# jcfaracco/xpysom-dask

Measured on AMD Instinct MI355X. Metric: samples/sec/epoch, higher is better.
Workload: dtype f16

## Files before the change

### xpysom_dask_amd/_lib.py

```python
import ctypes as C
import importlib.util
import os

HERE = os.path.dirname(os.path.abspath(__file__))
LIB_PATH = os.environ.get("SOM_LIB_PATH") or os.path.join(HERE, "libsomhip.so")

SOM_DIST = {"euclidean": 0, "euclidean_no_opt": 1, "cosine": 2, "manhattan": 3, "manhattan_no_opt": 3,
            "norm_p": 4, "norm_p_no_opt": 5}
SOM_NEIGH = {"gaussian": 0, "mexican_hat": 1, "bubble": 2, "triangle": 3}
SOM_PREC = {"f32": 0, "bf16": 1, "f16": 3, "exact": 5}
SOM_TOPO = {"rectangular": 0, "hexagonal": 1}
SOM_BMU_ACTIVATION, SOM_BMU_QUANTIZATION = 0, 1
SOM_KERNELS = {"bmu": 0, "segsum": 1, "kron": 2, "merge": 3, "prep": 4, "screen": 5}


class SomConfig(C.Structure):
    _fields_ = [("x", C.c_int32), ("y", C.c_int32), ("input_len", C.c_int32),
                ("distance", C.c_int32), ("neighborhood", C.c_int32),
                ("compact_support", C.c_int32), ("precision", C.c_int32), ("device", C.c_int32),
                ("std_coeff", C.c_double), ("stream", C.c_void_p),
                ("topology", C.c_int32), ("norm_p", C.c_int32), ("norm_p_real", C.c_double)]


_F = C.POINTER(C.c_float)
_I = C.POINTER(C.c_int32)
_H = C.c_void_p

SIGNATURES = {
    "som_version": (C.c_char_p, []),
    "som_device_count": (C.c_int, []),
    "som_last_error": (C.c_char_p, [_H]),
    "som_create": (C.c_int, [C.POINTER(SomConfig), C.POINTER(_H)]),
    "som_destroy": (None, [_H]),
    "som_set_weights": (C.c_int, [_H, _F]),
    "som_get_weights": (C.c_int, [_H, _F]),
    "som_set_data": (C.c_int, [_H, _F, C.c_int64]),
    "som_set_data_device": (C.c_int, [_H, C.c_void_p, C.c_int64]),
    "som_sync_producer": (C.c_int, [_H, C.c_uint64, C.c_int32]),
    "som_copy_to_host": (C.c_int, [_H, C.c_void_p, C.c_uint64, C.c_void_p]),
    "som_epoch_accumulate": (C.c_int, [_H, C.c_double, C.c_double, C.c_int]),
    "som_epoch_accumulate_faithful": (C.c_int, [_H, C.c_double, C.c_double, C.c_int]),
    "som_epoch_merge": (C.c_int, [_H]),
    "som_epoch": (C.c_int, [_H, C.c_double, C.c_double, C.c_int]),
    "som_epoch_accumulate_begin": (C.c_int, [_H, C.c_double, C.c_double, C.c_int]),
    "som_epoch_block_count": (C.c_int, [_H, C.POINTER(C.c_int32)]),
    "som_epoch_accumulate_block": (C.c_int, [_H, C.c_int32, C.POINTER(C.c_int64), C.POINTER(C.c_int64)]),
    "som_comm_load": (C.c_int, [C.c_char_p]),
    "som_comm_unique_id": (C.c_int, [C.c_void_p]),
    "som_comm_init": (C.c_int, [_H, C.c_int32, C.c_int32, C.c_void_p]),
    "som_epoch_allreduce": (C.c_int, [_H]),
    "som_comm_destroy": (C.c_int, [_H]),
    "som_pinned_alloc": (C.c_int, [C.c_uint64, C.POINTER(C.c_void_p)]),
    "som_pinned_free": (C.c_int, [C.c_void_p]),
    "som_stream_begin": (C.c_int, [_H]),
    "som_stream_rows": (C.c_int, [_H, _F, C.c_int64]),
    "som_stream_end": (C.c_int, [_H, C.c_double, C.c_double, C.c_int]),
    "som_accum_device_ptr": (C.c_int, [_H, C.POINTER(C.c_void_p), C.POINTER(C.c_int64)]),
    "som_get_stream": (C.c_int, [_H, C.POINTER(C.c_void_p)]),
    "som_epoch_fetch": (C.c_int, [_H, _F, _F, _I]),
    "som_epoch_accumulate_forced": (C.c_int, [_H, _I, C.c_double, C.c_double, C.c_int]),
    "som_bmu": (C.c_int, [_H, _F, C.c_int64, C.c_int32, _I]),
    "som_bmu_device": (C.c_int, [_H, C.c_void_p, C.c_int64, C.c_int32, _I]),
    "som_bmu_top2": (C.c_int, [_H, _F, C.c_int64, _I, _I]),
    "som_bmu_top2_device": (C.c_int, [_H, C.c_void_p, C.c_int64, _I, _I]),
    "som_bmu_f64": (C.c_int, [_H, C.POINTER(C.c_double), C.c_int64, _I]),
    "som_distance_matrix": (C.c_int, [_H, _F, C.c_int64, C.c_int32, _F]),
    "som_quantization_error": (C.c_int, [_H, _F, C.c_int64, C.POINTER(C.c_double)]),
    "som_quantization_error_device": (C.c_int, [_H, C.c_void_p, C.c_int64, C.POINTER(C.c_double)]),
    "som_set_verify": (C.c_int, [_H, C.c_int32]),
    "som_verify_stats": (C.c_int, [_H, C.POINTER(C.c_int64), C.POINTER(C.c_int64)]),
    "som_debug_corrupt_operands": (C.c_int, [_H, C.c_int32]),
    "som_debug_operand_crc": (C.c_int, [_H, C.c_int32, C.POINTER(C.c_uint64)]),
    "som_debug_exact_centroids": (C.c_int, [_H, C.c_int32, _F, _F, _F, _I]),
    "som_debug_mfma16": (C.c_int, [_H, C.c_void_p, C.c_void_p, _F, _F, C.c_int32]),
    "som_debug_stamps": (C.c_int, [_H, C.c_int64, C.c_void_p]),
    "som_debug_device_bytes": (C.c_int, [C.POINTER(C.c_int64)]),
    "som_debug_qe_stats": (C.c_int, [_H, C.POINTER(C.c_int64), C.POINTER(C.c_int64)]),
    "som_debug_exact_chain_stats": (C.c_int, [_H, C.POINTER(C.c_int64)]),
    "som_debug_exact_select_stats": (C.c_int, [_H, C.POINTER(C.c_int64), C.POINTER(C.c_int64), C.POINTER(C.c_int64)]),
    "som_policy_eval": (C.c_int, [C.c_int32, C.POINTER(C.c_double), C.POINTER(C.c_double), C.POINTER(C.c_int32)]),
    "som_policy_replay": (C.c_int, [C.c_int32, C.POINTER(C.c_double), C.POINTER(C.c_double)]),
    "som_patch_order": (C.c_int, [C.c_int32, C.c_int32, _I]),
    "som_exact_stats": (C.c_int, [_H, C.POINTER(C.c_int64), C.POINTER(C.c_int64), C.POINTER(C.c_int64)]),
    "som_exact_top2_stats": (C.c_int, [_H, C.POINTER(C.c_int64), C.POINTER(C.c_int64)]),
    "som_exact_skip_stats": (C.c_int, [_H, C.POINTER(C.c_int64), C.POINTER(C.c_int64)]),
    "som_exact_resident_stats": (C.c_int, [_H, C.POINTER(C.c_int64), C.POINTER(C.c_int64)]),
    "som_exact_scout_stats": (C.c_int, [_H, C.POINTER(C.c_int64), C.POINTER(C.c_int64)]),
    "som_exact_refine_stats": (C.c_int, [_H, C.POINTER(C.c_int64), C.POINTER(C.c_int64)]),
    "som_exact_last_counts": (C.c_int, [_H, _I, C.c_int64]),
    "som_sync": (C.c_int, [_H]),
    "som_profile_enable": (C.c_int, [_H, C.c_int32]),
    "som_profile_get": (C.c_int, [_H, C.c_int32, C.POINTER(C.c_double), C.POINTER(C.c_int64)]),
    "som_profile_reset": (C.c_int, [_H]),
}

_lib = None


def torch_lib_file(name):
    try:
        spec = importlib.util.find_spec("torch")
    except (ImportError, ValueError):
        spec = None
    if spec is None or not spec.submodule_search_locations:
        return None
    cand = os.path.join(list(spec.submodule_search_locations)[0], "lib", name)
    return cand if os.path.exists(cand) else None


def _preload_torch_hip_runtime():
    try:
        spec = importlib.util.find_spec("torch")
    except (ImportError, ValueError):
        spec = None
    if spec is None or not spec.submodule_search_locations:
        return
    cand = os.path.join(list(spec.submodule_search_locations)[0], "lib", "libamdhip64.so")
    if os.path.exists(cand):
        try:
            C.CDLL(cand, mode=C.RTLD_GLOBAL)
        except OSError:
            pass


def load():
    global _lib
    if _lib is not None:
        return _lib
    if not os.path.exists(LIB_PATH):
        raise ImportError(
            f"{LIB_PATH} is missing: build it with `python -m xpysom_dask_amd.build` "
            "(needs hipcc; there is no CPU fallback)")
    if not os.environ.get("SOM_LIB_PATH"):
        from . import build as _build
        have, want = _build.built_hash(LIB_PATH), _build.source_hash()
        if have != want:
            raise ImportError(
                f"{LIB_PATH} is stale: built from sources {have}, the tree is {want}; "
                "rebuild with `python -m xpysom_dask_amd.build`")
    _preload_torch_hip_runtime()
    lib = C.CDLL(LIB_PATH)
    for name, (res, args) in SIGNATURES.items():
        fn = getattr(lib, name)
        fn.restype = res
        fn.argtypes = args
    _lib = lib
    return lib
```

### xpysom_dask_amd/csrc/exact_host.hpp

```cpp

struct PassCtr {
    int* base; int n_groups; bool whole_lines;
    int* gcount() const { return base; }
    int* gstart() const { return base + n_groups; }
    PassCounters* tail() const { return (PassCounters*)(gstart() + n_groups); }
    RowNeed* row_need() const { return (RowNeed*)base; }
    size_t bytes() const {
        const size_t b = 2 * (size_t)n_groups * sizeof(int) + sizeof(PassCounters);
        return whole_lines ? (size_t)round_up((long)b, 64) : b;
    }
};
constexpr size_t EX_CTR_TAIL_INTS = (sizeof(PassCounters) + 64) / sizeof(int);
inline PassCtr pass_ctr(const som_handle* h) { return PassCtr{h->ex.ctr, (int)cdiv(h->K, EX_GROUP), h->ex.chain}; }

constexpr double EX_KAPPA = 6.0;
ExactBound exact_bound(const som_handle* h) {
    const double u = std::ldexp(1.0, -24);
    const double Dl = h->wide ? 32.0 * h->ft_kchunks : 8.0 * h->fr_kg;
    const double n_mfma = h->wide ? h->n_kchunks : h->ks32;
    const double gamma = Dl * u / (1.0 - Dl * u);
    const double slop = 1.01;
    ExactBound eb{};
    eb.cB = (float)(slop * 2.0 * (EX_KAPPA * n_mfma + 1.0) * std::ldexp(1.0, -23));
    eb.cM = (float)(slop * 2.0);
// ... 244 lines not shown
    ex.tile_counts.reset(); ex.tlist.reset(); ex.tcnt.reset(); ex.scout_g.reset(); ex.items.reset(); ex.tile_ticket.reset();
    ex.sk_stride = 0;
    const long tiles = stride / SK_TILE;
    if (int rc = ex.sk_keys.alloc(h, (size_t)stride)) return rc;
    if (int rc = ex.sk_keys2.alloc(h, (size_t)stride)) return rc;
    if (int rc = ex.sk_vals.alloc(h, (size_t)stride)) return rc;
    if (int rc = ex.scout_g.alloc(h, (size_t)stride)) return rc;
    if (h->wide)
        if (int rc = ex.tq.alloc(h, (size_t)stride)) return rc;
    if (int rc = ex.need.alloc(h, (size_t)tiles * ex.cen[0].n_cstages)) return rc;
    if (int rc = ex.need2.alloc(h, (size_t)tiles * ex.cen[1].n_cstages)) return rc;
    if (int rc = ex.glist.alloc(h, (size_t)tiles * n_groups)) return rc;
    if (int rc = ex.gcnt.alloc(h, (size_t)tiles)) return rc;
    if (int rc = ex.tile_counts.alloc(h, (size_t)tiles)) return rc;
    if (int rc = ex.tlist.alloc(h, (size_t)tiles * n_groups * K16_T)) return rc;
    if (int rc = ex.tcnt.alloc(h, (size_t)tiles)) return rc;
    if (int rc = ex.tile_ticket.alloc(h, (size_t)tiles)) return rc;
    ex.item_slots = (int)resident_slots(h, 8);
    if (int rc = ex.items.alloc(h, (size_t)(5 * tiles + 4 * ex.item_slots + 16))) return rc;
    if (int rc = ex.sk_tmp.alloc(h, radix_scratch_ints(stride))) return rc;
    ex.sk_stride = stride;
    return 0;
}

template <class E>
int exact_skip_centroids(som_handle* h, const float* xmax2, unsigned q_blocks, unsigned long long* best64, long n_rows, bool* q_done) {
    auto& ex = h->ex;
    const float* Wsrc = h->ex_patch ? h->Wp : h->W;
    const int n_groups = (int)cdiv(h->K, EX_GROUP);
    auto& c0 = ex.cen[0];
    auto& c1 = ex.cen[1];
    const CentroidLevel l1{c0.Cc, c0.rg, c0.csq, c0.cmax2, c0.n_slots}, l2{c1.Cc, c1.rg, c1.csq, c1.cmax2, c1.n_slots};
    if (!ex.cen_fresh)
        exact_centroids_kernel<<<dim3((unsigned)(cdiv(n_groups, 4) * 4)), dim3(512), 0, h->stream>>>(Wsrc, h->K, h->D, n_groups, l1, l2, h->wmax2);
    const int nst2 = ex.lp.level2 ? c1.n_cstages : 0;
    char* plain = ex.lp.scout ? c0.Cst_plain : nullptr;
    const dim3 tgrid((unsigned)cdiv((long)(c0.n_cstages + nst2) * K16_T, 4)), block(256);
    if (ex.prep_w_pending) {
        ex.prep_w_pending = false;
        const float* Wex = h->ex_patch ? h->Wp : h->W;
        float* cm1 = ex.prep_w_cm ? (float*)c0.cmax2 : nullptr;
        float* cm2 = ex.prep_w_cm ? (float*)c1.cmax2 : nullptr;
        const unsigned w_blocks = (unsigned)cdiv((long)h->n_stages * K16_T, 4);
        switch (h->ks32) {
#define SOM_PIMG_CASE(k) case k: exact_prep_images_kernel<k, E><<<dim3(w_blocks + tgrid.x + q_blocks), block, 0, h->stream>>>(w_blocks, tgrid.x, Wex, h->K, h->D, h->Wst, h->n_stages, \
            h->wmax2 + 1, h->Wst_lo, cm1, cm2, l1, c0.Cst, c0.n_cstages, l2, c1.Cst, nst2, xmax2, h->wmax2, plain, h->wn, h->stage_units, best64, n_rows); break;
        SOM_PIMG_CASE(1) SOM_PIMG_CASE(2) SOM_PIMG_CASE(3) SOM_PIMG_CASE(4)
#undef SOM_PIMG_CASE
        default: return fail(h, "exact: block skipping supports input_len <= 128");
        }
        HIPCHK(h, hipGetLastError());
        *q_done = q_blocks > 0;
        return 0;
    }
    switch (h->ks32) {
#define SOM_CIMG_CASE(k) case k: exact_centroid_image_kernel<k, E><<<tgrid, block, 0, h->stream>>>(l1, c0.Cst, c0.n_cstages, l2, c1.Cst, nst2, h->D, xmax2, h->wmax2, plain); break;
    SOM_CIMG_CASE(1) SOM_CIMG_CASE(2) SOM_CIMG_CASE(3) SOM_CIMG_CASE(4)
#undef SOM_CIMG_CASE
    default: return fail(h, "exact: block skipping supports input_len <= 128");
    }
    HIPCHK(h, hipGetLastError());
    return 0;
}

int exact_skip_sortkeys(som_handle* h, som_handle::ExactScratch::SortedRows& sr, long s0, long n, const int* prev, const int* scout_g) {
    auto& ex = h->ex;
    const int n_groups = (int)cdiv(h->K, EX_GROUP);
    if (scout_g != nullptr)
        exact_groupkey_kernel<<<dim3((unsigned)cdiv(n, 256)), dim3(256), 0, h->stream>>>(scout_g, n, n_groups, ex.sk_keys, ex.sk_vals);
    else
        exact_sortkey_kernel<<<dim3((unsigned)cdiv(n, 256)), dim3(256), 0, h->stream>>>(prev, h->ex_inv, n, h->K, ex.sk_keys, ex.sk_vals);
    int bits = 1;
    while ((1L << bits) < n_groups) ++bits;
    return radix_sort_rows(h, ex.sk_keys, n, bits, ex.sk_keys2, sr.order + s0, ex.sk_tmp);
}
template <class E>
int exact_skip_gather(som_handle* h, som_handle::ExactScratch::SortedRows& sr, long s0, const int* order, const float* X, const __bf16* Xb, long n,
                      const float* xsq, const float* xerr, const float* xmax2) {
    const long np = round_up(n, SK_TILE);
    exact_gather_sorted_kernel<E><<<dim3((unsigned)cdiv(np, 16)), dim3(256), 0, h->stream>>>(
        order, n, np, h->dp, h->D, Xb, X, xsq, xerr, xmax2, sr.Xb_s + s0 * h->dp, sr.Xl_s != nullptr ? sr.Xl_s + s0 * h->dp : nullptr, sr.Xf_s + s0 * h->D,
        sr.xsq_s + s0, sr.xerr_s + s0);
    HIPCHK(h, hipGetLastError());
    return 0;
}

template <int KS32, class E>
int exact_scout_nearest_ks(som_handle* h, const __bf16* Xb, long n, unsigned long long* best64, int* g_out) {
    auto& ex = h->ex;
    const auto& c0 = ex.cen[0];
    const void* kern = (const void*)bmu_bf16_k16_kernel<KS32, E, false, false>;
    const size_t lds = 2 * (size_t)k16_stage_bytes(KS32);
    int per_cu = 1;
    if (int rc = kernel_per_cu(h, kern, 64 * K16_NW, lds, &per_cu)) return rc;
    const long blocks = cdiv(n, K16_WG_SAMPLES);
    const long slots = resident_slots(h, per_cu);
    const int parts = std::max(1, std::min(choose_parts(h, blocks, slots, c0.n_cstages), c0.n_cstages));
    bmu_bf16_k16_kernel<KS32, E, false, false><<<dim3((unsigned)blocks, (unsigned)parts), dim3(64 * K16_NW), lds, h->stream>>>(
        Xb, n, c0.Cst_plain, c0.n_cstages, c0.n_slots, best64);
    bmu_finalize_kernel<<<dim3((unsigned)cdiv(n, 256)), dim3(256), 0, h->stream>>>(best64, n, c0.n_slots, g_out);
    HIPCHK(h, hipMemsetAsync(best64, 0xFF, (size_t)n * sizeof(unsigned long long), h->stream));
    HIPCHK(h, hipGetLastError());
    return 0;
}
template <class E>
int exact_scout_nearest(som_handle* h, const __bf16* Xb, long n, unsigned long long* best64, int* g_out) {
    SOM_KS32_DISPATCH(exact_scout_nearest_ks, h, Xb, n, best64, g_out)
    return fail(h, "exact: the scout supports input_len <= 128");
}

template <int KS32, class E>
int exact_scout_pick_ks(som_handle* h, som_handle::ExactScratch::SortedRows& sr, long s0, long n, const int* keys, unsigned long long* best64) {
    auto& ex = h->ex;
    const int n_groups = (int)cdiv(h->K, EX_GROUP);
    const long tiles = round_up(n, SK_TILE) / SK_TILE;
    const size_t lds_l = (size_t)cdiv(n_groups, 64) * sizeof(unsigned long long);
    exact_scout_lists_kernel<<<dim3((unsigned)tiles), dim3(64), lds_l, h->stream>>>(keys, nullptr, n, n_groups, ex.tlist, ex.tcnt);
    const void* kern = (const void*)bmu_bf16_k16_kernel<KS32, E, false, true>;
    const size_t lds = 2 * (size_t)k16_stage_bytes(KS32);
    int per_cu = 1;
    if (int rc = kernel_per_cu(h, kern, 64 * K16_NW, lds, &per_cu)) return rc;
    bmu_bf16_k16_kernel<KS32, E, false, true><<<dim3((unsigned)tiles, 1), dim3(64 * K16_NW), lds, h->stream>>>(
        sr.Xb_s + s0 * h->dp, n, h->Wst, h->n_stages, h->K, best64, nullptr, 0, nullptr, nullptr, nullptr, nullptr, nullptr, nullptr, ExactBound(),
        nullptr, ex.tlist, ex.tcnt);
    exact_scout_pos_kernel<<<dim3((unsigned)cdiv(n, 256)), dim3(256), 0, h->stream>>>(best64, n, h->K, sr.lastpos_s + s0);
    HIPCHK(h, hipGetLastError());
    return 0;
}
template <class E>
int exact_scout_pick(som_handle* h, som_handle::ExactScratch::SortedRows& sr, long s0, long n, const int* keys, unsigned long long* best64) {
    SOM_KS32_DISPATCH(exact_scout_pick_ks, h, sr, s0, n, keys, best64)
    return fail(h, "exact: the scout supports input_len <= 128");
}

void exact_plan_lists(som_handle* h, long tiles, int n_cstages, const unsigned long long* need2) {
    auto& ex = h->ex;
    const int n_groups = (int)cdiv(h->K, EX_GROUP);
    PassCounters* const ctr = pass_ctr(h).tail();
    const int slots = ex.item_queue ? (ex.screen_slots > 0 ? ex.screen_slots : ex.item_slots) : 0;
    int2* const queue = ex.item_queue ? ex.items + 8 : nullptr;
    int* const n_items = (int*)ex.items.p;
    if (ex.chain) {
        exact_lists_totals_kernel<<<dim3((unsigned)cdiv(tiles, LISTS_WG_TILES)), dim3(64 * LISTS_WG_TILES), 0, h->stream>>>(
            ex.need, n_cstages, need2, n_groups, ex.glist, ex.gcnt, ex.tile_counts, ex.tlist, ex.tcnt, tiles, &ctr->lists_done,
            &ctr->blocks_run, &ctr->groups_run, slots, queue, n_items, n_items + 1, ex.item_len_pct, ex.tile_ticket);
        return;
    }
    exact_lists_kernel<<<dim3((unsigned)tiles), dim3(64), 0, h->stream>>>(ex.need, n_cstages, need2, n_groups, ex.glist, ex.gcnt,
                                                                         ex.tile_counts, ex.tlist, ex.tcnt, ex.tile_ticket);
    exact_list_totals_kernel<<<dim3(1), dim3(1024), 0, h->stream>>>(ex.tile_counts, tiles, &ctr->blocks_run, &ctr->groups_run, slots, queue,
                                                                  n_items, n_items + 1, ex.item_len_pct);
}

template <class E>
int exact_skip_plan(som_handle* h, som_handle::ExactScratch::SortedRows& sr, long s0, long n, const float* xmax2, const ExactBound& eb,
                    const int* lastpos2, bool time_l2 = false) {
    auto& ex = h->ex;
    PassCounters* const ctr = pass_ctr(h).tail();
    const long np = round_up(n, SK_TILE);
    const long tiles = np / SK_TILE;
    const dim3 block(64 * K16_NW);
    const auto& c0 = ex.cen[0];
    const auto& c1 = ex.cen[1];
    const long want = (1024 + tiles - 1) / tiles;
    const dim3 pgrid((unsigned)tiles, (unsigned)std::max<long>(1, std::min<long>({want, 4L, (long)c0.n_cstages})));
    const size_t lds1 = 2 * (size_t)h->stage_bytes + (size_t)c0.n_cstages * 8;
    const size_t lds2 = 2 * (size_t)h->stage_bytes + (size_t)c0.n_cstages * 64 * sizeof(int) + (size_t)c1.n_cstages * 8;
    const bool l2 = ex.lp.level2;
    const int force = ex.skip_mode == 3 ? 1 : 0;
    const __bf16* Xs = sr.Xb_s + s0 * h->dp;
    unsigned long long* const need2_clear = l2 && ex.chain ? ex.need2.p : nullptr;
    if (l2 && !ex.chain) HIPCHK(h, hipMemsetAsync(ex.need2, 0, (size_t)tiles * c1.n_cstages * sizeof(unsigned long long), h->stream));
#define SOM_PLAN_CASE(k) case k: { \
        { int pc; if (int rc = kernel_per_cu(h, (const void*)exact_plan_kernel<k, E, false>, 64 * K16_NW, lds1, &pc)) return rc; } \
        exact_plan_kernel<k, E, false><<<pgrid, block, lds1, h->stream>>>(Xs, n, c0.Cst, c0.n_cstages, c0.rg, c0.n_slots, \
            sr.xsq_s + s0, sr.xerr_s + s0, sr.sU_s + s0, xmax2, c0.cmax2, h->wmax2, h->wmax2 + 1, eb, ex.need, sr.lastpos_s + s0, \
            h->Wst, sr.seed_s + s0, nullptr, 0, force, lastpos2, lastpos2 != nullptr ? &ctr->scout_wins : nullptr, need2_clear); \
        if (l2) { \
            if (time_l2) (void)hipEventRecord(ex.cost.ev[3], h->stream); \
            { int pc; if (int rc = kernel_per_cu(h, (const void*)exact_plan_kernel<k, E, true>, 64 * K16_NW, lds2, &pc)) return rc; } \
            exact_plan_kernel<k, E, true><<<dim3((unsigned)tiles, pgrid.y), block, lds2, h->stream>>>(Xs, n, c1.Cst, c1.n_cstages, c1.rg, c1.n_slots, \
                sr.xsq_s + s0, sr.xerr_s + s0, sr.sU_s + s0, xmax2, c1.cmax2, h->wmax2, h->wmax2 + 1, eb, ex.need2, nullptr, \
                nullptr, nullptr, ex.need, c0.n_cstages, force); \
            if (time_l2) (void)hipEventRecord(ex.cost.ev[4], h->stream); \
        } } break;
    switch (h->ks32) {
    SOM_PLAN_CASE(1) SOM_PLAN_CASE(2) SOM_PLAN_CASE(3) SOM_PLAN_CASE(4)
    default: return fail(h, "exact: block skipping supports input_len <= 128");
    }
#undef SOM_PLAN_CASE
    exact_plan_lists(h, tiles, c0.n_cstages, l2 ? ex.need2.p : nullptr);
    HIPCHK(h, hipGetLastError());
    return 0;
}

template <class E>
int exact_wide_centroids(som_handle* h, const float* xmax2) {
    auto& ex = h->ex;
    auto& c0 = ex.cen[0];
    const float* Wsrc = h->ex_patch ? h->Wp : h->W;
    const int n_groups = (int)cdiv(h->K, EX_GROUP);
    wide_centroids_kernel<<<dim3((unsigned)n_groups), dim3(256), 0, h->stream>>>(Wsrc, h->K, h->D, n_groups, c0.Cc, c0.rg, c0.csq, c0.cmax2, h->wmax2);
    const long total = (long)c0.n_img_stages * WD_T * h->n_kchunks * 64;
    prep_w_bf16_wide_kernel<E><<<dim3((unsigned)cdiv(total, 256)), dim3(256), 0, h->stream>>>(c0.Cc, n_groups, h->D, h->n_kchunks, c0.Cst, c0.n_img_stages,
                                                                                             nullptr, h->wmax2);
    exact_werr_kernel<E><<<dim3((unsigned)cdiv(n_groups, 4 * EX_WERR_UNITS)), dim3(256), 0, h->stream>>>(c0.Cc, n_groups, h->D, h->wmax2, c0.cmax2 + 1, nullptr);
    char* plain = ex.lp.scout ? c0.Cst_plain : nullptr;
    if (plain) HIPCHK(h, hipMemcpyAsync(plain, c0.Cst, (size_t)c0.n_img_stages * h->stage_bytes, hipMemcpyDeviceToDevice, h->stream));
    wide_centroid_tail_kernel<<<dim3((unsigned)cdiv((long)c0.n_img_stages * WD_STAGE_UNITS, 256)), dim3(256), 0, h->stream>>>(
        c0.rg, c0.csq, n_groups, c0.Cst, c0.n_img_stages, h->stage_bytes, xmax2, h->wmax2, plain);
    HIPCHK(h, hipGetLastError());
    return 0;
}

template <class E>
int exact_wide_gather(som_handle* h, som_handle::ExactScratch::SortedRows& sr, long s0, const float* X, long n, const float* xsq, const float* xerr,
                      const int* prev, const float* xmax2) {
    const long np = round_up(n, SK_TILE);
    wide_gather_sorted_kernel<<<dim3((unsigned)cdiv(np, 4)), dim3(256), 0, h->stream>>>(sr.order + s0, n, np, h->D, X, xsq, xerr, prev,
                                                                                      sr.Xf_s + s0 * h->D, sr.xsq_s + s0, sr.xerr_s + s0, sr.lastpos_s + s0);
    const long n_blocks = np / h->tl_bm;
    const long total = n_blocks * h->n_kchunks * (h->tl_bm / 16) * TL_KS * 64;
    prep_tiles_bf16_kernel<E><<<dim3((unsigned)cdiv(total, 256)), dim3(256), 0, h->stream>>>(
        sr.Xf_s + s0 * h->D, n, h->D, h->n_kchunks, n_blocks, h->tl_bm, h->tl_xtile, 1.0f, nullptr, (char*)(sr.Xb_s + s0 * h->dp), xmax2);
    HIPCHK(h, hipGetLastError());
    return 0;
}

template <int KS32, class E>
int exact_wide_scout_nearest_ks(som_handle* h, const __bf16* Ximg, long n, unsigned long long* best64, int* g_out) {
    auto& ex = h->ex;
    const auto& c0 = ex.cen[0];
    const size_t lds = (size_t)WD_SLOTS * wd_stage_bytes(KS32);
    int per_cu = 1;
    if (int rc = kernel_per_cu(h, (const void*)bmu_bf16_wide_kernel<KS32, E>, 64 * WD_NW, lds, &per_cu)) return rc;
    const long blocks = cdiv(n, WD_WG_SAMPLES);
    const long slots = resident_slots(h, per_cu);
    const int parts = (int)std::max<long>(1, std::min<long>({cdiv(2 * slots, blocks), 8L, (long)c0.n_img_stages}));
    bmu_bf16_wide_kernel<KS32, E><<<dim3((unsigned)blocks, (unsigned)parts), dim3(64 * WD_NW), lds, h->stream>>>(
        (const char*)Ximg, n, c0.Cst_plain, c0.n_img_stages, best64);
    bmu_finalize_kernel<<<dim3((unsigned)cdiv(n, 256)), dim3(256), 0, h->stream>>>(best64, n, c0.n_slots, g_out);
    HIPCHK(h, hipMemsetAsync(best64, 0xFF, (size_t)n * sizeof(unsigned long long), h->stream));
    HIPCHK(h, hipGetLastError());
    return 0;
}
template <int KS32, class E>
int exact_wide_scout_pick_ks(som_handle* h, som_handle::ExactScratch::SortedRows& sr, long s0, long n, const int* keys, unsigned long long* best64) {
    auto& ex = h->ex;
    const int n_groups = (int)cdiv(h->K, EX_GROUP);
    const long tiles = round_up(n, SK_TILE) / SK_TILE;
    const size_t lds_l = (size_t)cdiv(n_groups, 64) * sizeof(unsigned long long);
    exact_scout_lists_kernel<<<dim3((unsigned)tiles), dim3(64), lds_l, h->stream>>>(keys, nullptr, n, n_groups, ex.glist, ex.gcnt, 1);
    const size_t lds = (size_t)WD_SLOTS * wd_stage_bytes(KS32);
    int per_cu = 1;
    if (int rc = kernel_per_cu(h, (const void*)bmu_bf16_wide_kernel<KS32, E, false, true>, 64 * WD_NW, lds, &per_cu)) return rc;
    bmu_bf16_wide_kernel<KS32, E, false, true><<<dim3((unsigned)tiles, 1), dim3(64 * WD_NW), lds, h->stream>>>(
        (const char*)(sr.Xb_s + s0 * h->dp), n, h->Wst, h->n_stages, best64, nullptr, 0, nullptr, nullptr, nullptr, nullptr, nullptr, nullptr, ExactBound(),
        ex.glist, ex.gcnt, n_groups);
    exact_scout_pos_kernel<<<dim3((unsigned)cdiv(n, 256)), dim3(256), 0, h->stream>>>(best64, n, h->K, sr.lastpos_s + s0, h->ex_perm);
    HIPCHK(h, hipGetLastError());
    return 0;
}
template <class E>
int exact_wide_scout_nearest(som_handle* h, const __bf16* Ximg, long n, unsigned long long* best64, int* g_out) {
    SOM_WIDE_DISPATCH(exact_wide_scout_nearest_ks, h, Ximg, n, best64, g_out)
    return fail(h, "exact: no wide scout instance for this input_len");
}
template <class E>
int exact_wide_scout_pick(som_handle* h, som_handle::ExactScratch::SortedRows& sr, long s0, long n, const int* keys, unsigned long long* best64) {
    SOM_WIDE_DISPATCH(exact_wide_scout_pick_ks, h, sr, s0, n, keys, best64)
    return fail(h, "exact: no wide scout instance for this input_len");
}

template <int KS32, class E>
int exact_wide_plan_ks(som_handle* h, som_handle::ExactScratch::SortedRows& sr, long s0, long n, const float* xmax2, const ExactBound& eb) {
    auto& ex = h->ex;
    const auto& c0 = ex.cen[0];
    const long np = round_up(n, SK_TILE);
    const long tiles = np / SK_TILE;
    exact_seed_kernel<<<dim3((unsigned)cdiv(n * 16, 256)), dim3(256), 0, h->stream>>>(
        sr.Xf_s + s0 * h->D, n, h->D, h->W, h->wsq, h->K, sr.lastpos_s + s0, sr.xsq_s + s0, sr.xerr_s + s0, h->wmax2, xmax2, h->wmax2 + 1, eb, ex.seed, ex.tq);
    wide_plan_rows_kernel<<<dim3((unsigned)cdiv(n, 256)), dim3(256), 0, h->stream>>>(n, sr.xsq_s + s0, sr.xerr_s + s0, ex.tq, xmax2, c0.cmax2, h->wmax2,
                                                                                  h->wmax2 + 1, eb, ex.skip_mode == 3 ? 1 : 0, sr.seed_s + s0, sr.sU_s + s0);
    HIPCHK(h, hipMemsetAsync(ex.need, 0, (size_t)tiles * c0.n_cstages * sizeof(unsigned long long), h->stream));
    auto kern = bmu_bf16_wide_kernel<KS32, E, false, false, true>;
    const size_t lds = (size_t)WD_SLOTS * wd_stage_bytes(KS32) + (size_t)c0.n_cstages * sizeof(unsigned long long);
    int per_cu = 1;
    if (int rc = kernel_per_cu(h, (const void*)kern, 64 * WD_NW, lds, &per_cu)) return rc;
    const long slots = resident_slots(h, per_cu);
    int parts = (int)std::max<long>(1, std::min<long>({cdiv(2 * slots, tiles), 8L, (long)c0.n_img_stages}));
    bmu_bf16_wide_kernel<KS32, E, false, false, true><<<dim3((unsigned)tiles, (unsigned)parts), dim3(64 * WD_NW), lds, h->stream>>>(
        (const char*)(sr.Xb_s + s0 * h->dp), n, c0.Cst, c0.n_img_stages, nullptr, nullptr, 0, nullptr, nullptr, nullptr, nullptr, nullptr, nullptr, ExactBound(),
        nullptr, nullptr, 0, sr.seed_s + s0, sr.sU_s + s0, ex.need, c0.n_cstages);
    exact_plan_lists(h, tiles, c0.n_cstages, nullptr);
    HIPCHK(h, hipGetLastError());
    return 0;
}
template <class E>
int exact_wide_plan(som_handle* h, som_handle::ExactScratch::SortedRows& sr, long s0, long n, const float* xmax2, const ExactBound& eb) {
    SOM_WIDE_DISPATCH(exact_wide_plan_ks, h, sr, s0, n, xmax2, eb)
    return fail(h, "exact: no wide plan instance for this input_len");
}

template <int KG>
int exact_rescore_kg(som_handle* h, const float* X, unsigned long long* best64, int deint) {
    auto& ex = h->ex;
    auto kern = exact_rescore_mfma_kernel<KG>;
    const size_t lds = (size_t)fr_stage_bytes(KG);
    int per_cu = 1;
    if (int rc = kernel_per_cu(h, (const void*)kern, 256, lds, &per_cu)) return rc;
    const long grid = std::min<long>(ex.max_tiles, h->ex.grid_mult * resident_slots(h, per_cu));
    kern<<<dim3((unsigned)grid), dim3(256), lds, h->stream>>>(X, h->D, h->Wfst, h->K, ex.tile_tab, &pass_ctr(h).tail()->n_tiles, ex.plist,
                                                             best64, h->ex_perm, nullptr, h->ex_sub44 ? 1 : 0, deint, nullptr);
    return 0;
}

inline unsigned exact_tiles_blocks(const som_handle* h) { return h->ex.chain ? 16u : 1u; }

template <int KS32, class E>
int exact_refine_ks(som_handle* h, som_handle::ExactScratch::SortedRows& sr, long r0, long n, const float* xmax2, const ExactBound& eb) {
    auto& ex = h->ex;
    const PassCtr pc = pass_ctr(h);
    const int n_groups = pc.n_groups;
// ... 385 lines not shown
```

### xpysom_dask_amd/csrc/exact_skip.hpp

```cpp
#pragma once
#include "bmu_bf16_k16.hpp"
#include "bmu_f32_res.hpp"

namespace somhip {

constexpr int SK_TILE = K16_WG_SAMPLES;
static_assert(K16_STAGE_UNITS == 64 && K16_T == 4, "block skipping: a stage of the resident screen is one 64-unit group of four 16-unit tiles");

struct CentroidLevel { float* C; float* rg; float* csq; float* cmax2; int n_slots; };
struct CentroidShared {
    float qsum[4][128];
    float part[2][64][2];
    float csq_s[2][5];
};
__device__ __forceinline__ void group_centroids(const float (&w)[16], int g, int K, int D, const CentroidLevel& l1,
                                                const CentroidLevel& l2, CentroidShared& sh) {
    const int tid = threadIdx.x, lane = tid & 63;
    const int d = tid & 127, q = tid >> 7, fh = (tid >> 6) & 1;
    const int cnt = (int)max(0L, min(64L, (long)K - (long)g * 64));
    const int cb = max(0, min(16, cnt - 16 * q));
    float sum = 0.0f;
#pragma unroll
    for (int k = 0; k < 16; ++k) sum += w[k];
    sh.qsum[q][d] = sum;
// ... 156 lines not shown

template <class EL>
__global__ __launch_bounds__(256) void exact_gather_sorted_kernel(const int* __restrict__ order, long n, long np, int dp, int D,
                                                                  const __bf16* __restrict__ Xb, const float* __restrict__ X,
                                                                  const float* __restrict__ xsq, const float* __restrict__ xerr,
                                                                  const float* __restrict__ xmax2,
                                                                  __bf16* __restrict__ Xb_s, __bf16* __restrict__ Xl_s,
                                                                  float* __restrict__ Xf_s,
                                                                  float* __restrict__ xsq_s, float* __restrict__ xerr_s) {
    using E = typename EL::T;
    using bf16x8 = typename V8<E>::t;
    const int lane = threadIdx.x & 15;
    const long p = (long)blockIdx.x * 16 + (threadIdx.x >> 4);
    if (p >= np) return;
    const long r = p < n ? (long)order[p] : -1;
    const float sx = ex_scale(*xmax2);
    const bool vec = (D & 7) == 0;
    for (int c = lane; c < dp / 8; c += 16) {
        bf16x8 v, vl;
#pragma unroll
        for (int j = 0; j < 8; ++j) { v[j] = (E)0.0f; vl[j] = (E)0.0f; }
        if (r >= 0) {
            v = *(const bf16x8*)((const char*)Xb + (r * dp + c * 8) * 2);
            float f[8];
            if (vec && c * 8 < D) {
                const f32x4 a = *(const f32x4*)(X + r * D + c * 8), b = *(const f32x4*)(X + r * D + c * 8 + 4);
                const f32x4 ev = {a[0], a[2], b[0], b[2]}, od = {a[1], a[3], b[1], b[3]};
                *(f32x4*)(Xf_s + p * D + c * 4) = ev;
                *(f32x4*)(Xf_s + p * D + D / 2 + c * 4) = od;
#pragma unroll
                for (int j = 0; j < 4; ++j) { f[j] = a[j]; f[4 + j] = b[j]; }
            } else {
#pragma unroll
                for (int j = 0; j < 8; ++j) {
                    f[j] = c * 8 + j < D ? X[r * D + c * 8 + j] : 0.0f;
                    if (c * 8 + j < D) Xf_s[p * D + c * 8 + j] = f[j];
                }
            }
#pragma unroll
            for (int j = 0; j < 8; ++j) {
                const float d = (f[j] * sx - (float)v[j]) * 2048.0f;
                vl[j] = cvt<E>(d == d && __builtin_fabsf(d) < 3.0e38f ? d : 0.0f);
            }
        }
        *(bf16x8*)((char*)Xb_s + (p * dp + c * 8) * 2) = v;
        if (Xl_s != nullptr) *(bf16x8*)((char*)Xl_s + (p * dp + c * 8) * 2) = vl;
    }
    if (lane == 0) {
        const float nanv = __builtin_nanf("");
        xsq_s[p] = r >= 0 ? xsq[r] : nanv;
        xerr_s[p] = r >= 0 ? xerr[r] : nanv;
    }
}

__device__ __forceinline__ float up_to_half(float v) {
    if (!(v == v)) return v;
    if (v > 65504.0f) return __builtin_inff();
    if (v < 0x1p-14f) return 0x1p-14f;
    const _Float16 hv = (_Float16)v;
    float f = (float)hv;
    if (f < v) f = (float)__builtin_bit_cast(_Float16, (unsigned short)(__builtin_bit_cast(unsigned short, hv) + 1));
    return f;
}

__device__ __forceinline__ uint32_t row16_or(uint32_t v) {
    v |= (uint32_t)__builtin_amdgcn_update_dpp(0, (int)v, 0x121, 0xF, 0xF, false);
    v |= (uint32_t)__builtin_amdgcn_update_dpp(0, (int)v, 0x122, 0xF, 0xF, false);
    v |= (uint32_t)__builtin_amdgcn_update_dpp(0, (int)v, 0x124, 0xF, 0xF, false);
    v |= (uint32_t)__builtin_amdgcn_update_dpp(0, (int)v, 0x128, 0xF, 0xF, false);
    return v;
}

template <int KS32, class EL>
__device__ __forceinline__ void exact_centroid_image_body(const unsigned bid, const CentroidLevel& l1, char* __restrict__ Cst1, int n_cstages1,
                                                          const CentroidLevel& l2, char* __restrict__ Cst2, int n_cstages2, int D,
                                                          const float* __restrict__ xmax2, const float* __restrict__ wmax2,
                                                          char* __restrict__ Cst1_plain) {
    using E = typename EL::T;
    using bf16x8 = typename V8<E>::t;
    constexpr int STAGE = k16_stage_bytes(KS32);
    const int lane = threadIdx.x & 63;
    long tile = (long)bid * 4 + (threadIdx.x >> 6);
    const long t1 = (long)n_cstages1 * K16_T;
    const bool second = tile >= t1;
    if (second) tile -= t1;
    if (tile >= (long)(second ? n_cstages2 : n_cstages1) * K16_T) return;
    const CentroidLevel& lv = second ? l2 : l1;
    char* Cst = second ? Cst2 : Cst1;
    const long stage = tile / K16_T;
    const int t16 = (int)(tile - stage * K16_T);
    const long slot = stage * K16_STAGE_UNITS + t16 * 16 + (lane & 15);
    const float sw = ex_scale(*wmax2), sx = ex_scale(*xmax2);
    float er = 0.0f;
#pragma unroll
    for (int ks = 0; ks < KS32; ++ks) {
        const int k0 = ks * 32 + (lane >> 4) * 8;
        bf16x8 v;
#pragma unroll
        for (int j = 0; j < 8; ++j) {
            const float f = (slot < lv.n_slots && k0 + j < D) ? lv.C[slot * D + k0 + j] * sw : 0.0f;
            const E hb = cvt<E>(-f);
            v[j] = hb;
            const float e = half_operand_error(-f, (float)hb);
            er = __builtin_fmaf(e, e, er);
        }
        *(bf16x8*)(Cst + stage * STAGE + ((long)(t16 * KS32 + ks) * 64 + lane) * 16) = v;
        if (!second && Cst1_plain != nullptr) *(bf16x8*)(Cst1_plain + stage * STAGE + ((long)(t16 * KS32 + ks) * 64 + lane) * 16) = v;
    }
    er += __shfl_xor(er, 16, 64);
    er += __shfl_xor(er, 32, 64);
    float m = (er == er) ? er : 0.0f;
#pragma unroll
    for (int o = 8; o > 0; o >>= 1) m = fmaxf(m, __shfl_xor(m, o, 64));
    if (lane == 0) atomic_max_pos_f32(lv.cmax2 + 1, m);
    if (lane < 16) {
        float* tail = (float*)(Cst + (stage + 1) * (long)STAGE - 1024);
        const int within = t16 * 16 + lane;
        const float rad = slot < lv.n_slots ? lv.rg[slot] : -1.0f;
        float* ptail = (!second && Cst1_plain != nullptr) ? (float*)(Cst1_plain + (stage + 1) * (long)STAGE - 1024) : nullptr;
        if (rad < 0.0f) { tail[within] = __builtin_inff(); tail[64 + within] = 0.0f; if (ptail) ptail[within] = __builtin_inff(); }
        else {
            const float big = __builtin_sqrtf(*wmax2) * __builtin_sqrtf(*xmax2) * (1.0f + 1.0f / 1024.0f);
            const float S = sx * sw, hS = 0.5f * S * (1.0f + 1.0f / 1024.0f);
            const float s0 = __builtin_fmaf(0.5f * S, lv.csq[slot], S * big);
            tail[within] = s0 - hS * rad * rad * (1.0f + 0x1p-20f);
            tail[64 + within] = -up_to_half(sw * rad);
            if (ptail) ptail[within] = (s0 == s0 && s0 < 3.0e38f) ? s0 : __builtin_inff();
        }
    }
}
template <int KS32, class EL>
__global__ __launch_bounds__(256) void exact_centroid_image_kernel(CentroidLevel l1, char* __restrict__ Cst1, int n_cstages1,
                                                                   CentroidLevel l2, char* __restrict__ Cst2, int n_cstages2, int D,
                                                                   const float* __restrict__ xmax2, const float* __restrict__ wmax2,
                                                                   char* __restrict__ Cst1_plain = nullptr) {
    exact_centroid_image_body<KS32, EL>(blockIdx.x, l1, Cst1, n_cstages1, l2, Cst2, n_cstages2, D, xmax2, wmax2, Cst1_plain);
}

template <int KS32, class EL>
__global__ __launch_bounds__(256) void exact_prep_images_kernel(unsigned w_blocks, unsigned c_blocks, const float* __restrict__ W, int K, int D,
                                                                char* __restrict__ Wst, int n_stages, float* __restrict__ werr2,
                                                                char* __restrict__ Wst_lo, float* __restrict__ cm1, float* __restrict__ cm2,
                                                                CentroidLevel l1, char* __restrict__ Cst1, int n_cstages1,
                                                                CentroidLevel l2, char* __restrict__ Cst2, int n_cstages2,
                                                                const float* __restrict__ xmax2, const float* __restrict__ wmax2,
                                                                char* __restrict__ Cst1_plain, const float* __restrict__ wn,
                                                                int stage_units, unsigned long long* __restrict__ best64, long n_rows) {
    if (blockIdx.x < w_blocks) prep_w_exact_k16_body<KS32, EL>(blockIdx.x, W, K, D, Wst, n_stages, wmax2, werr2, Wst_lo, cm1, cm2, false);
    else if (blockIdx.x < w_blocks + c_blocks)
        exact_centroid_image_body<KS32, EL>(blockIdx.x - w_blocks, l1, Cst1, n_cstages1, l2, Cst2, n_cstages2, D, xmax2, wmax2, Cst1_plain);
    else prep_wsqh_body(blockIdx.x - w_blocks - c_blocks, wn, K, wmax2, xmax2, Wst, n_stages, k16_stage_bytes(KS32), stage_units, best64, n_rows, 1);
}

template <int KS32, class EL, bool LEVEL2>
__global__ __launch_bounds__(64 * K16_NW, LEVEL2 ? 3 : 2) void exact_plan_kernel(const __bf16* __restrict__ Xb, long N,
                                                                    const char* __restrict__ Cst, int n_cstages,
                                                                    const float* __restrict__ rg, int n_slots,
                                                                    const float* __restrict__ xsq, const float* __restrict__ xerr,
                                                                    float* __restrict__ sU_s,
                                                                    const float* __restrict__ xmax2, const float* __restrict__ cmax2,
                                                                    const float* __restrict__ wmax2, const float* __restrict__ werr2,
                                                                    ExactBound eb, unsigned long long* __restrict__ need,
                                                                    const int* __restrict__ lastpos, const char* __restrict__ Wst,
                                                                    float* __restrict__ seed_s,
                                                                    const unsigned long long* __restrict__ need1, int n_cstages1,
                                                                    int force_all, const int* __restrict__ lastpos2 = nullptr,
                                                                    int* __restrict__ scout_wins = nullptr,
                                                                    unsigned long long* __restrict__ need2_clear = nullptr) {
    using E = typename EL::T;
    using bf16x8 = typename V8<E>::t;
    constexpr int DP = 32 * KS32;
    constexpr int STAGE = k16_stage_bytes(KS32);
    constexpr int PIECES = K16_T * KS32 + 1;
    extern __shared__ __attribute__((aligned(16))) char smem[];
    __shared__ int act_n;

    const int tid = threadIdx.x, lane = tid & 63;
    const int wave = __builtin_amdgcn_readfirstlane(tid >> 6);
    const int quad = lane >> 4, col = lane & 15;
    const long wave_s0 = (long)blockIdx.x * K16_WG_SAMPLES + wave * (16 * K16_SB);

    bf16x8 xf[K16_SB][KS32];
    bf16x8 xe[K16_SB];
    float A[K16_SB], sU[K16_SB], P[K16_SB];
    const ExactScales sc = ex_scales(xmax2, cmax2, cmax2 + 1);
    const ExactScales sw = ex_scales(xmax2, wmax2, werr2);
    const float S = sc.sx * sc.sw;
#pragma unroll
    for (int sb = 0; sb < K16_SB; ++sb) {
        const long row = wave_s0 + sb * 16 + col;
#pragma unroll
        for (int ks = 0; ks < KS32; ++ks) xf[sb][ks] = *(const bf16x8*)(Xb + row * DP + ks * 32 + quad * 8);
        A[sb] = -__builtin_inff(); sU[sb] = 0.0f;
        if (row < N) {
            const float q = xsq[row], xe = xerr[row];
            float su;
            if (!LEVEL2) {
                auto value_of = [&](int pos) -> float {
                    const char* stg = Wst + (long)(pos >> 6) * STAGE;
                    const int t16 = (pos >> 4) & 3, c = pos & 15;
                    float d = 0.0f;
#pragma unroll
                    for (int ks = 0; ks < KS32; ++ks) {
                        const bf16x8 a = *(const bf16x8*)(stg + ((t16 * KS32 + ks) * 64 + quad * 16 + c) * 16);
#pragma unroll
                        for (int jj = 0; jj < 8; ++jj) d = __builtin_fmaf((float)a[jj], (float)xf[sb][ks][jj], d);
                    }
                    d += __shfl_xor(d, 16, 64);
                    d += __shfl_xor(d, 32, 64);
                    return *(const float*)(stg + K16_T * KS32 * 1024 + (t16 * 16 + c) * 4) + d;
                };
                float vu = value_of(lastpos[row]);
                if (lastpos2 != nullptr) {
                    const float v2 = value_of(lastpos2[row]);
                    const float Sq = sw.sx * sw.sw;
                    const float ua = q + 2.0f * (vu / Sq - sw.big), ub = q + 2.0f * (v2 / Sq - sw.big);
                    const bool win = ua < 0.9f * ub;
                    const unsigned long long wm = __ballot(win && quad == 0);
                    if (scout_wins != nullptr && lane == __builtin_ctzll(__ballot(true)) && wm != 0ull) atomicAdd(scout_wins, (int)__popcll(wm));
                    vu = (v2 < vu || !(vu == vu)) ? v2 : vu;
                }
                const float Sw = sw.sx * sw.sw;
                const float e = ex_row_bound(eb, sw, q, xe);
                const float f32s = ex_f32_share(eb, sw, q);
                const float e_valu = 48.0f * 0x1p-24f * Sw * sw.bmag;
                const float sd = vu + (e - f32s) * (1.0f + 1.0f / 1024.0f) + e_valu + Sw * sw.bmag * 0x1p-21f;
                if (quad == 0) seed_s[row] = (sd > 0.0f && sd < 3.0e38f) ? sd : __builtin_inff();
                const float e_one = 0.5f * (e - f32s) * (1.0f + 1.0f / 1024.0f) + e_valu;
                const float tau_up = 2.0f * (((vu + e_one) - Sw * sw.big) / Sw) + 0x1p-20f * (sw.big + __builtin_fabsf(vu) / Sw);
                const float xn = __builtin_sqrtf(q) * (1.0f + 1.0f / 1024.0f);
                const float share = 2.0f * (eb.cA * xn * sw.wm + eb.cW * sw.wm * sw.wm);
                const float U0 = q * (1.0f + 1.0f / 1024.0f) + tau_up + share * (1.0f + 1.0f / 1024.0f) + 0x1p-18f * (q + __builtin_fabsf(tau_up));
                const float U = U0 < 0.0f ? 0.0f : U0;
                su = __builtin_sqrtf(U) * (1.0f + 1.0f / 1024.0f);
                if (force_all || !(su == su) || !(su < 3.0e38f) || !(e == e)) su = __builtin_inff();
                if (quad == 0) sU_s[row] = su;
            } else {
                su = sU_s[row];
            }
            const float ec = 0.5f * ex_row_bound(eb, sc, q, xe) * (1.0f + 1.0f / 1024.0f);
            sU[sb] = su;
            A[sb] = S * sc.big + ec - 0.5f * S * q * (1.0f - 1.0f / 1024.0f) + 0x1p-12f * S * (sc.big + q) + 0x1p-16f * S * sc.wm * sc.wm;
            if (!(A[sb] == A[sb]) || !(A[sb] < 3.0e38f) || !(su < 3.0e38f)) {
                A[sb] = __builtin_inff(); sU[sb] = 0.0f;
            }
        }
        const float bx = up_to_half(sc.sx * sU[sb] * (1.0f + 1.0f / 1024.0f));
        P[sb] = A[sb] + 0.5f * S * (1.0f + 1.0f / 1024.0f) * sU[sb] * sU[sb] * (1.0f + 0x1p-20f) + (float)(24 * (KS32 + 1)) * 0x1p-23f * S * sc.bmag;
        if (!(bx < 3.0e38f) || !(P[sb] == P[sb])) P[sb] = __builtin_inff();
        if (A[sb] == -__builtin_inff()) P[sb] = -__builtin_inff();
#pragma unroll
        for (int jj = 0; jj < 8; ++jj) xe[sb][jj] = (E)0.0f;
        if (quad == 0 && bx < 3.0e38f) xe[sb][0] = (E)bx;
    }

    int* act = (int*)(smem + 2 * STAGE);
    unsigned long long* nl = (unsigned long long*)(smem + 2 * STAGE + (LEVEL2 ? (size_t)n_cstages1 * 64 * sizeof(int) : 0));
    for (int i = tid; i < n_cstages; i += 64 * K16_NW) nl[i] = 0ull;
    if constexpr (LEVEL2) {
        static_assert(K16_NW == 4, "a wave per tile fills the slot's tail");
        if (wave == 0) {
            int cnt = 0;
            for (int s1 = 0; s1 < n_cstages1; ++s1) {
                const unsigned long long w = need1[(long)blockIdx.x * n_cstages1 + s1];
                const int g = s1 * 64 + lane;
                const bool on = ((w >> lane) & 1ull) && 4 * (g >> 2) * 4 < n_slots;
                const unsigned long long mk = __ballot(on);
                if (on) act[cnt + __popcll(mk & ((1ull << lane) - 1ull))] = g;
                cnt += __popcll(mk);
            }
            if (lane == 0) act_n = cnt;
        }
        __syncthreads();
        const int n_act = act_n;
        const int c_all = (n_act + 15) / 16;
        const int b0 = 16 * (int)((long)c_all * blockIdx.y / gridDim.y);
        const int e0 = min(n_act, 16 * (int)((long)c_all * (blockIdx.y + 1) / gridDim.y));
        constexpr int TQ = K16_T * KS32 * 1024;
        auto frag_of = [&](int g, int sub, int ks, int q) -> const char* {
            return Cst + (long)(g >> 4) * STAGE + (((((g >> 2) & 3) * KS32 + ks) * 64 + q * 16 + 4 * (g & 3) + sub) * 16);
        };
        auto dma_chunk = [&](int c0, char* dst) {
            for (int p = wave; p < K16_T * KS32; p += K16_NW) {
                const int j = p / KS32, ks = p - j * KS32;
                if (c0 + 4 * j < e0) {
                    const int gi = c0 + 4 * j + (col >> 2);
                    const int g = gi < e0 ? act[gi] : act[c0 + 4 * j];
                    lds_dma_16(frag_of(g, col & 3, ks, quad), dst + p * 1024);
                }
            }
        };
        auto load_tail = [&](int c0) -> float {
            const int i = lane & 15, gi = c0 + 4 * wave + (i >> 2);
            if (lane >= 32 || gi >= e0) return lane < 16 ? __builtin_inff() : 0.0f;
            const int g = act[gi];
            return *(const float*)(Cst + (long)(g >> 4) * STAGE + TQ + (((lane >> 4) * 64) + ((g >> 2) & 3) * 16 + 4 * (g & 3) + (i & 3)) * 4);
        };
        auto store_tail = [&](char* dst, float v) {
            if (lane < 32) *(float*)(dst + TQ + (((lane >> 4) * 64) + wave * 16 + (lane & 15)) * 4) = v;
        };
        if (b0 < e0) { dma_chunk(b0, smem); store_tail(smem, load_tail(b0)); }
        int k = 0;
        for (int c0 = b0; c0 < e0; c0 += 16, ++k) {
            asm volatile("s_waitcnt vmcnt(0) lgkmcnt(0)" ::: "memory");
            __builtin_amdgcn_s_barrier();
            asm volatile("" ::: "memory");
            char* sn = smem + ((k + 1) & 1) * STAGE;
            float tail_n = 0.0f;
            if (c0 + 16 < e0) { dma_chunk(c0 + 16, sn); tail_n = load_tail(c0 + 16); }
            const char* st = smem + (k & 1) * STAGE;
            const float* wq = (const float*)(st + TQ);
            auto load_tile = [&](int j, bf16x8 (&a)[KS32], f32x4& wv, float& rneg) {
#pragma unroll
                for (int ks = 0; ks < KS32; ++ks) a[ks] = *(const bf16x8*)(st + ((j * KS32 + ks) * 64 + lane) * 16);
                wv = *(const f32x4*)(wq + j * 16 + 4 * quad);
                rneg = wq[64 + j * 16 + col];
            };
            uint32_t lane_bits = 0u;
            auto run_tile = [&](int j, const bf16x8 (&a)[KS32], const f32x4& wv, float rneg) {
                bf16x8 ae;
#pragma unroll
                for (int jj = 0; jj < 8; ++jj) ae[jj] = (E)0.0f;
                if (quad == 0) ae[0] = (E)rneg;
                f32x4 acc[K16_SB];
#pragma unroll
                for (int sb = 0; sb < K16_SB; ++sb) acc[sb] = wv;
#pragma unroll
                for (int ks = 0; ks < KS32; ++ks)
#pragma unroll
                    for (int sb = 0; sb < K16_SB; ++sb) acc[sb] = mfma16(a[ks], xf[sb][ks], acc[sb]);
#pragma unroll
                for (int sb = 0; sb < K16_SB; ++sb) acc[sb] = mfma16(ae, xe[sb], acc[sb]);
#pragma unroll
                for (int r = 0; r < 4; ++r) {
                    bool nd = false;
#pragma unroll
                    for (int sb = 0; sb < K16_SB; ++sb) nd = nd || !(acc[sb][r] > P[sb]);
                    lane_bits |= nd ? (1u << (4 * j + r)) : 0u;
                }
            };
            bf16x8 aA[KS32], aB[KS32];
            f32x4 wvA, wvB;
            float rnA, rnB;
            const bool h1 = c0 + 4 < e0, h2 = c0 + 8 < e0, h3 = c0 + 12 < e0;
            load_tile(0, aA, wvA, rnA);
            if (h1) load_tile(1, aB, wvB, rnB);
            run_tile(0, aA, wvA, rnA);
            if (h1) {
                if (h2) load_tile(2, aA, wvA, rnA);
                run_tile(1, aB, wvB, rnB);
                if (h2) {
                    if (h3) load_tile(3, aB, wvB, rnB);
                    run_tile(2, aA, wvA, rnA);
                    if (h3) run_tile(3, aB, wvB, rnB);
                }
            }
            const uint32_t any_row = row16_or(lane_bits);
            if (col == 0 && any_row != 0u) {
#pragma unroll
                for (int j = 0; j < 4; ++j) {
                    const uint32_t nib = (any_row >> (4 * j)) & 15u;
                    const int gi = c0 + 4 * j + quad;
                    if (nib != 0u && gi < e0) {
                        const int g = act[gi];
                        atomicOr(nl + (g >> 4), (unsigned long long)nib << (4 * (g & 15)));
                    }
                }
            }
            if (c0 + 16 < e0) store_tail(sn, tail_n);
        }
        __syncthreads();
        for (int i = tid; i < n_cstages; i += 64 * K16_NW)
            if (nl[i] != 0ull) atomicOr(need + (long)blockIdx.x * n_cstages + i, nl[i]);
        return;
    }
    const int n_walk = n_cstages;
    const int s_begin = (int)((long)n_walk * blockIdx.y / gridDim.y);
    const int s_end = (int)((long)n_walk * (blockIdx.y + 1) / gridDim.y);
    auto item_of = [&](int i) -> int { return (i << 4) | 15; };
    auto dma_stage = [&](int s, uint32_t tm, char* dst) {
        const char* src = Cst + (long)s * STAGE;
        for (int p = wave; p < PIECES; p += K16_NW)
            if (p == PIECES - 1 || ((tm >> (p / KS32)) & 1u)) lds_dma_16(src + (long)p * 1024 + lane * 16, dst + p * 1024);
    };
    int st_cur = 0, st_next = 0;
    uint32_t tm_cur = 0, tm_next = 0;
    if (s_begin < s_end) {
        const int it = item_of(s_begin);
        st_cur = it >> 4; tm_cur = (uint32_t)it & 15u;
        dma_stage(st_cur, tm_cur, smem);
    }
    for (int i = s_begin; i < s_end; ++i) {
        asm volatile("s_waitcnt vmcnt(0) lgkmcnt(0)" ::: "memory");
        __builtin_amdgcn_s_barrier();
        asm volatile("" ::: "memory");
        if (i + 1 < s_end) {
            const int it = item_of(i + 1);
            st_next = it >> 4; tm_next = (uint32_t)it & 15u;
            dma_stage(st_next, tm_next, smem + ((i + 1 - s_begin) & 1) * STAGE);
        }
        const char* st = smem + ((i - s_begin) & 1) * STAGE;
        const float* wq = (const float*)(st + K16_T * KS32 * 1024);
        uint32_t lane_bits = 0u;
        auto load_tile = [&](int t, bf16x8 (&a)[KS32], f32x4& wv, float& rneg) {
#pragma unroll
            for (int ks = 0; ks < KS32; ++ks) a[ks] = *(const bf16x8*)(st + ((t * KS32 + ks) * 64 + lane) * 16);
            wv = *(const f32x4*)(wq + t * 16 + 4 * quad);
            rneg = wq[64 + t * 16 + col];
        };
        auto run_tile = [&](int t16, const bf16x8 (&a)[KS32], const f32x4& wv, float rneg) {
            bf16x8 ae;
#pragma unroll
            for (int jj = 0; jj < 8; ++jj) ae[jj] = (E)0.0f;
            if (quad == 0) ae[0] = (E)rneg;
            f32x4 acc[K16_SB];
#pragma unroll
            for (int sb = 0; sb < K16_SB; ++sb) acc[sb] = wv;
#pragma unroll
            for (int ks = 0; ks < KS32; ++ks)
#pragma unroll
                for (int sb = 0; sb < K16_SB; ++sb) acc[sb] = mfma16(a[ks], xf[sb][ks], acc[sb]);
#pragma unroll
            for (int sb = 0; sb < K16_SB; ++sb) acc[sb] = mfma16(ae, xe[sb], acc[sb]);
#pragma unroll
            for (int r = 0; r < 4; ++r) {
                bool nd = false;
#pragma unroll
                for (int sb = 0; sb < K16_SB; ++sb) nd = nd || !(acc[sb][r] > P[sb]);
                lane_bits |= nd ? (1u << (4 * t16 + r)) : 0u;
            }
        };
        const uint32_t m0 = 15u, m1 = m0 & (m0 - 1u), m2 = m1 & (m1 - 1u), m3 = m2 & (m2 - 1u);
        const int t0 = __builtin_ctz(m0), t1 = m1 ? __builtin_ctz(m1) : -1, t2 = m2 ? __builtin_ctz(m2) : -1, t3 = m3 ? __builtin_ctz(m3) : -1;
        bf16x8 aA[KS32], aB[KS32];
        f32x4 wvA, wvB;
        float rnA, rnB;
        load_tile(t0, aA, wvA, rnA);
        if (t1 >= 0) load_tile(t1, aB, wvB, rnB);
        run_tile(t0, aA, wvA, rnA);
        if (t1 >= 0) {
            if (t2 >= 0) load_tile(t2, aA, wvA, rnA);
            run_tile(t1, aB, wvB, rnB);
            if (t2 >= 0) {
                if (t3 >= 0) load_tile(t3, aB, wvB, rnB);
                run_tile(t2, aA, wvA, rnA);
                if (t3 >= 0) run_tile(t3, aB, wvB, rnB);
            }
        }
        const uint32_t any_row = row16_or(lane_bits);
        if (col == 0 && any_row != 0u) {
            const uint32_t lo = ((any_row & 15u) | (((any_row >> 4) & 15u) << 16)) << (4 * quad);
            const uint32_t hi = (((any_row >> 8) & 15u) | (((any_row >> 12) & 15u) << 16)) << (4 * quad);
            atomicOr(nl + (i - s_begin), ((unsigned long long)hi << 32) | lo);
        }
        st_cur = st_next; tm_cur = tm_next;
    }
    __syncthreads();
    for (int i = s_begin + tid; i < s_end; i += 64 * K16_NW) need[(long)blockIdx.x * n_cstages + i] = nl[i - s_begin];
    if (need2_clear != nullptr)
        for (int i = 4 * s_begin + tid; i < 4 * s_end; i += 64 * K16_NW) need2_clear[(long)blockIdx.x * 4 * n_cstages + i] = 0ull;
}

template <bool PUBLISH>
__device__ __forceinline__ void exact_lists_tile(const long tile, const int lane, const unsigned long long* __restrict__ need1, int n_cstages,
                                                 const unsigned long long* __restrict__ need2, int n_groups,
                                                 int* __restrict__ glist, int* __restrict__ gcnt,
                                                 int2* tile_counts, int* __restrict__ tlist,
                                                 int* __restrict__ tcnt, int* __restrict__ tile_ticket) {
    const unsigned long long below = (1ull << lane) - 1ull;
    int base = 0, blk = 0, kept = 0;
    for (int s0 = 0; s0 < n_cstages; s0 += 64) {
        const unsigned long long mine = s0 + lane < n_cstages ? need1[tile * n_cstages + s0 + lane] : 0ull;
        const uint32_t lo = (uint32_t)mine, hi = (uint32_t)(mine >> 32);
        unsigned long long todo = __ballot(mine != 0ull);
        for (; todo != 0ull; todo &= todo - 1ull) {
            const int sl = (int)__builtin_ctzll(todo), s = s0 + sl;
            const unsigned long long w = ((unsigned long long)(uint32_t)__builtin_amdgcn_readlane((int)hi, sl) << 32) |
                                         (uint32_t)__builtin_amdgcn_readlane((int)lo, sl);
            uint32_t nib = 15u;
            if (need2 != nullptr) nib = (uint32_t)(need2[tile * 4 * n_cstages + 4 * s + (lane >> 4)] >> (4 * (lane & 15))) & 15u;
            const int g = s * 64 + lane;
            const bool l1 = ((w >> lane) & 1ull) && g < n_groups;
            const bool on = l1 && nib != 0u;
            const unsigned long long mk = __ballot(on);
            if (on) glist[tile * n_groups + base + __popcll(mk & ((1ull << lane) - 1ull))] = (g << 4) | (int)nib;
            base += __popcll(mk);
            kept += __popcll(__ballot(l1));
            int before = 0, total = 0;
#pragma unroll
            for (int b = 0; b < 4; ++b) {
                const unsigned long long mb = __ballot(on && ((nib >> b) & 1u));
                before += __popcll(mb & below);
                total += __popcll(mb);
            }
            if (on) {
                int o = blk + before;
#pragma unroll
                for (int b = 0; b < 4; ++b)
                    if ((nib >> b) & 1u) tlist[tile * 4 * n_groups + o++] = (g << 2) | b;
            }
            blk += total;
        }
    }
    if (lane == 0) {
        gcnt[tile] = base; tcnt[tile] = blk;
        tile_ticket[tile] = 0;
        if (PUBLISH)
            __hip_atomic_store((unsigned long long*)(tile_counts + tile), ((unsigned long long)(uint32_t)kept << 32) | (uint32_t)blk,
                               __ATOMIC_RELAXED, __HIP_MEMORY_SCOPE_AGENT);
        else tile_counts[tile] = make_int2(blk, kept);
    }
}
__global__ __launch_bounds__(64) void exact_lists_kernel(const unsigned long long* __restrict__ need1, int n_cstages,
                                                         const unsigned long long* __restrict__ need2, int n_groups,
                                                         int* __restrict__ glist, int* __restrict__ gcnt,
                                                         int2* __restrict__ tile_counts, int* __restrict__ tlist,
                                                         int* __restrict__ tcnt, int* __restrict__ tile_ticket) {
    exact_lists_tile<false>(blockIdx.x, threadIdx.x, need1, n_cstages, need2, n_groups, glist, gcnt, tile_counts, tlist, tcnt, tile_ticket);
}

__device__ __forceinline__ void exact_list_totals_body(const int2* tile_counts, long tiles, int* __restrict__ blocks_run,
                                                       int* __restrict__ groups_run, int slots, int2* __restrict__ items,
                                                       int* __restrict__ n_items, int* __restrict__ item_ctr, int len_pct,
                                                       int* sb, int* sk, int& tot_b) {
    const int tid = threadIdx.x, lane = tid & 63, wave = tid >> 6;
    int b = 0, k = 0;
    for (long t = tid; t < tiles; t += 1024) { const int2 c = tile_counts[t]; b += c.x; k += c.y; }
#pragma unroll
    for (int o = 32; o > 0; o >>= 1) { b += __shfl_xor(b, o, 64); k += __shfl_xor(k, o, 64); }
    if (lane == 0) { sb[wave] = b; sk[wave] = k; }
    __syncthreads();
    if (tid == 0) {
        b = 0; k = 0;
        for (int w = 0; w < 16; ++w) { b += sb[w]; k += sk[w]; }
        *blocks_run = b; *groups_run = k;
        tot_b = b;
    }
    if (items == nullptr) return;
    __syncthreads();
    const long total = tot_b;
    const long by_mean = (len_pct * total) / (100 * (tiles > 0 ? tiles : 1)) + 1, by_slots = total / (2 * (long)(slots > 0 ? slots : 1));
    const int L = (int)max(32L, min(by_mean, by_slots));
    auto parts_of = [&](int cnt) -> int { return cnt <= L ? 1 : (cnt + L - 1) / L; };
    const long per = (tiles + 1023) / 1024, t_b = min((long)tid * per, tiles), t_e = min(t_b + per, tiles);
    int mine = 0;
    for (long t = t_b; t < t_e; ++t) mine += parts_of(tile_counts[t].x);
    int incl = mine;
#pragma unroll
    for (int o = 1; o < 64; o <<= 1) { const int v = __shfl_up(incl, o, 64); if (lane >= o) incl += v; }
    __syncthreads();
    if (lane == 63) sb[wave] = incl;
    __syncthreads();
    int before = 0, all = 0;
#pragma unroll
    for (int w = 0; w < 16; ++w) { if (w < wave) before += sb[w]; all += sb[w]; }
    int o = before + incl - mine;
    for (long t = t_b; t < t_e; ++t) {
        const int np = parts_of(tile_counts[t].x);
        for (int q = 0; q < np; ++q) items[o++] = make_int2((int)t, q | (np << 16));
    }
    if (tid == 0) { *n_items = all; *item_ctr = 0; }
}
__global__ __launch_bounds__(1024) void exact_list_totals_kernel(const int2* __restrict__ tile_counts, long tiles, int* __restrict__ blocks_run,
                                                                 int* __restrict__ groups_run, int slots = 0, int2* __restrict__ items = nullptr,
                                                                 int* __restrict__ n_items = nullptr, int* __restrict__ item_ctr = nullptr,
                                                                 int len_pct = 125) {
    __shared__ int sb[16], sk[16];
    __shared__ int tot_b;
    exact_list_totals_body(tile_counts, tiles, blocks_run, groups_run, slots, items, n_items, item_ctr, len_pct, sb, sk, tot_b);
}

constexpr int LISTS_WG_TILES = 16;
__global__ __launch_bounds__(64 * LISTS_WG_TILES) void exact_lists_totals_kernel(const unsigned long long* __restrict__ need1, int n_cstages,
                                                                                const unsigned long long* __restrict__ need2, int n_groups,
                                                                                int* __restrict__ glist, int* __restrict__ gcnt,
                                                                                int2* tile_counts, int* __restrict__ tlist,
                                                                                int* __restrict__ tcnt, long tiles, int* __restrict__ done,
                                                                                int* __restrict__ blocks_run, int* __restrict__ groups_run,
                                                                                int slots, int2* __restrict__ items, int* __restrict__ n_items,
                                                                                int* __restrict__ item_ctr, int len_pct,
                                                                                int* __restrict__ tile_ticket) {
    static_assert(LISTS_WG_TILES == 16, "the totals' scan is written for sixteen waves");
    __shared__ int sb[16], sk[16];
    __shared__ int tot_b;
    __shared__ int last;
    const int tid = threadIdx.x;
    const long tile = (long)blockIdx.x * LISTS_WG_TILES + (tid >> 6);
    if (tile < tiles) exact_lists_tile<true>(tile, tid & 63, need1, n_cstages, need2, n_groups, glist, gcnt, tile_counts, tlist, tcnt, tile_ticket);
    asm volatile("s_waitcnt vmcnt(0)" ::: "memory");
    __syncthreads();
    if (tid == 0) {
        const int ticket = __hip_atomic_fetch_add(done, 1, __ATOMIC_RELAXED, __HIP_MEMORY_SCOPE_AGENT);
        last = ticket == (int)gridDim.x - 1 ? 1 : 0;
        if (last) {
            __builtin_amdgcn_fence(__ATOMIC_ACQUIRE, "agent");
            asm volatile("s_waitcnt vmcnt(0)" ::: "memory");
            __hip_atomic_store(done, 0, __ATOMIC_RELAXED, __HIP_MEMORY_SCOPE_AGENT);
        }
    }
    __syncthreads();
    if (!last) return;
    exact_list_totals_body(tile_counts, tiles, blocks_run, groups_run, slots, items, n_items, item_ctr, len_pct, sb, sk, tot_b);
}

__global__ __launch_bounds__(256) void exact_groupkey_kernel(const int* __restrict__ g, long n, int n_groups, int* __restrict__ keys,
                                                             int* __restrict__ vals) {
    const long i = (long)blockIdx.x * 256 + threadIdx.x;
    if (i >= n) return;
    const int v = g[i];
    keys[i] = v < 0 ? 0 : v >= n_groups ? n_groups - 1 : v;
    vals[i] = (int)i;
}

__global__ __launch_bounds__(64) void exact_scout_lists_kernel(const int* __restrict__ gkey, const int* __restrict__ lastpos, long n,
                                                               int n_groups, int* __restrict__ tlist, int* __restrict__ tcnt,
                                                               int group_items = 0) {
    extern __shared__ unsigned long long sbm[];
    const long tile = blockIdx.x;
    const int lane = threadIdx.x;
    const int nw = (n_groups + 63) / 64;
    for (int w = lane; w < nw; w += 64) sbm[w] = 0ull;
    __syncthreads();
    for (int i = 0; i < SK_TILE / 64; ++i) {
        const long p = tile * SK_TILE + i * 64 + lane;
        if (p < n) {
            int g = gkey[p];
            g = g < 0 ? 0 : g >= n_groups ? n_groups - 1 : g;
            atomicOr(sbm + (g >> 6), 1ull << (g & 63));
            if (lastpos != nullptr) {
                int g2 = lastpos[p] >> 6;
                g2 = g2 < 0 ? 0 : g2 >= n_groups ? n_groups - 1 : g2;
                atomicOr(sbm + (g2 >> 6), 1ull << (g2 & 63));
            }
        }
    }
    __syncthreads();
    int base = 0;
    int* out = tlist + tile * (group_items ? 1 : 4) * (long)n_groups;
    for (int w0 = 0; w0 < nw; w0 += 64) {
        unsigned long long word = w0 + lane < nw ? sbm[w0 + lane] : 0ull;
        const int c = __popcll(word);
        int incl = c;
#pragma unroll
        for (int o = 1; o < 64; o <<= 1) { const int t = __shfl_up(incl, o, 64); if (lane >= o) incl += t; }
        int at = base + incl - c;
        for (; word != 0ull; word &= word - 1ull) {
            const int g = (w0 + lane) * 64 + (int)__builtin_ctzll(word);
            if (group_items) out[at] = (g << 4) | 15;
            else {
#pragma unroll
                for (int b = 0; b < 4; ++b) out[4 * at + b] = (g << 2) | b;
            }
            ++at;
        }
        base += __shfl(incl, 63, 64);
    }
    if (lane == 0) tcnt[tile] = group_items ? base : 4 * base;
}

__global__ __launch_bounds__(256) void exact_scout_rowneed_kernel(const float* __restrict__ X, long N, int D, int n_samples,
                                                                  const float* __restrict__ Cc, const float* __restrict__ rg,
                                                                  int n_groups, int* __restrict__ counts) {
    extern __shared__ float xs[];
    __shared__ float wmin[4];
    __shared__ int wcnt[4];
    const int tid = threadIdx.x, lane = tid & 63, wave = tid >> 6;
    const long step = N / n_samples;
    const float* x = X + ((long)blockIdx.x * step + step / 2) * D;
    for (int k = tid; k < D; k += 256) xs[k] = x[k];
    __syncthreads();
    auto dist = [&](int g) -> float {
        const float* c = Cc + (long)g * D;
        float q = 0.0f;
        if ((D & 3) == 0) {
            for (int k = 0; k < D; k += 4) {
                const f32x4 v = *(const f32x4*)(c + k);
#pragma unroll
                for (int j = 0; j < 4; ++j) { const float t = xs[k + j] - v[j]; q = __builtin_fmaf(t, t, q); }
            }
        } else {
            for (int k = 0; k < D; ++k) { const float t = xs[k] - c[k]; q = __builtin_fmaf(t, t, q); }
        }
        return __builtin_sqrtf(q);
    };
    float m = __builtin_inff();
    for (int g = tid; g < n_groups; g += 256) {
        const float r = rg[g];
        if (r >= 0.0f) m = __builtin_fminf(m, dist(g) + r);
    }
#pragma unroll
    for (int o = 32; o > 0; o >>= 1) m = __builtin_fminf(m, __shfl_xor(m, o, 64));
    if (lane == 0) wmin[wave] = m;
    __syncthreads();
    m = __builtin_fminf(__builtin_fminf(wmin[0], wmin[1]), __builtin_fminf(wmin[2], wmin[3]));
    int need = 0;
    for (int g = tid; g < n_groups; g += 256) {
        const float r = rg[g];
        if (r >= 0.0f) need += !(dist(g) - r > m) ? 1 : 0;
    }
#pragma unroll
    for (int o = 32; o > 0; o >>= 1) need += __shfl_xor(need, o, 64);
    if (lane == 0) wcnt[wave] = need;
    __syncthreads();
    if (tid == 0) { atomicAdd(counts, wcnt[0] + wcnt[1] + wcnt[2] + wcnt[3]); atomicAdd(counts + 1, 1); }
}

__global__ __launch_bounds__(256) void exact_sample_tiles_kernel(const int* __restrict__ order, const int* __restrict__ keys, long stride_tiles,
                                                                 int* __restrict__ order_out, int* __restrict__ keys_out) {
    const long src = (long)blockIdx.x * stride_tiles * SK_TILE + threadIdx.x;
    const long dst = (long)blockIdx.x * SK_TILE + threadIdx.x;
    static_assert(SK_TILE == 256, "one thread per row of a tile");
    order_out[dst] = order[src];
    keys_out[dst] = keys[src];
}

__global__ __launch_bounds__(256) void exact_scout_pos_kernel(unsigned long long* __restrict__ best64, long n, int K,
                                                              int* __restrict__ lastpos, const int* __restrict__ perm = nullptr) {
    const long p = (long)blockIdx.x * 256 + threadIdx.x;
    if (p >= n) return;
    const uint32_t u = (uint32_t)best64[p];
    const int pos = u < (uint32_t)K ? (int)u : 0;
    lastpos[p] = perm != nullptr ? perm[pos] : pos;
    best64[p] = ~0ull;
}

}
```

### xpysom_dask_amd/csrc/somhip.hip

```cpp
#include <hip/hip_runtime.h>

#include <cstring>

#include <dlfcn.h>

#include <cmath>
#include <cstdio>
#include <cstdlib>
#include <algorithm>
#include <atomic>
#include <cstring>
#include <string>
#include <utility>
#include <vector>

#include "../../include/somhip.h"
#include "../../include/somhip_test.h"
#include "bmu_bf16_k16.hpp"
#include "bmu_bf16_tiled.hpp"
#include "bmu_bf16_wide.hpp"
#include "bmu_exact.hpp"
#include "exact_skip.hpp"
#include "exact_policy.hpp"
#include "exact_skip_wide.hpp"
#include "bmu_f32.hpp"
#include "bmu_f32_res.hpp"
#include "bmu_f32_tiled.hpp"
#include "bmu_pairwise.hpp"
#include "update.hpp"

using namespace somhip;

namespace {

thread_local std::string g_create_error;

const char* dev_env(const char* name) {
    static const bool on = [] { const char* v = std::getenv("SOM_TEST_HOOKS"); return v != nullptr && std::atoi(v) != 0; }();
    return on ? std::getenv(name) : nullptr;
}

struct EventPair { hipEvent_t a, b; int kernel; };

}

struct som_nccl_id { char internal[128]; };
struct RcclApi {
    void* lib = nullptr;
    int (*GetUniqueId)(som_nccl_id*) = nullptr;
    int (*CommInitRank)(void**, int, som_nccl_id, int) = nullptr;
    int (*AllReduce)(const void*, void*, size_t, int, int, void*, hipStream_t) = nullptr;
    int (*CommDestroy)(void*) = nullptr;
    const char* (*GetErrorString)(int) = nullptr;
};
static RcclApi g_rccl;
static std::string g_rccl_error;

static std::atomic<int64_t> g_dev_bytes{0};
template <typename T>
struct DevBuf {
    T* p = nullptr;
    size_t cap = 0;
    DevBuf() = default;
    DevBuf(const DevBuf&) = delete;
    DevBuf& operator=(const DevBuf&) = delete;
    DevBuf(DevBuf&& o) noexcept : p(o.p), cap(o.cap) { o.p = nullptr; o.cap = 0; }
    DevBuf& operator=(DevBuf&& o) noexcept {
        if (this != &o) { reset(); p = o.p; cap = o.cap; o.p = nullptr; o.cap = 0; }
        return *this;
    }
    ~DevBuf() { reset(); }
    void reset() {
        if (p) { (void)hipFree(p); g_dev_bytes -= (int64_t)(cap * sizeof(T)); }
        p = nullptr; cap = 0;
    }
    int alloc(som_handle* h, size_t n);
    int reserve(som_handle* h, size_t n, size_t round = 1) { return n <= cap ? 0 : alloc(h, (n + round - 1) / round * round); }
    operator T*() const { return p; }
};

struct som_handle {
    som_config cfg{};
    void* comm = nullptr;
    int comm_world = 1;
    hipStream_t comm_stream = nullptr;
    hipEvent_t ev_block = nullptr, ev_comm = nullptr;
    int X = 0, Y = 0, K = 0, D = 0, D1p = 0;
    int ks32 = 0;
    bool tiled = false;
    bool f16 = false;
    bool exact = false;
    bool ex_patch = false, wf_patch = false;
    bool ex_sub44 = false;
    DevBuf<int> ex_perm;
    DevBuf<int> ex_inv;
    DevBuf<float> Wp;
    DevBuf<float> wsq_p;
    struct ExactScratch {
        DevBuf<uint32_t> gmin;
        DevBuf<unsigned long long> gflags;
        long stride = 0;
        DevBuf<int> rowcnt;
        DevBuf<int> rowarg;
        DevBuf<float> seed;
        bool seed_on = true;
        bool seed_live = false;
        int two_round = -1;
        DevBuf<int> fb_list, fb_ids;
        DevBuf<int> ctr;
        DevBuf<int> plist;
        DevBuf<int4> tile_tab;
        long max_tiles = 0;
        DevBuf<float> fbX;
        PassCounters* pass_host = nullptr;
        hipEvent_t fb_ready = nullptr;
        int64_t rows_total = 0, rows_fallback = 0, chunks = 0;
        int64_t blocks_run = 0, blocks_total = 0;
        long pass_rows_override = 0;
        long hook_refuse_above = 0, hook_pairs = 0; bool hook_refuse_skip = false;
        long stride_cap = 0;
        long pairs = 64;
        int skip_mode = 1;
        policy::PlanState plan;
        policy::LaunchPlan lp;
        bool sub_blocks = true;
        struct SortedRows {
            long cap = 0;
            DevBuf<int> order;
            DevBuf<__bf16> Xb_s;
            DevBuf<__bf16> Xl_s;
            bool xl_filled = false;
            DevBuf<float> Xf_s, xsq_s, xerr_s, seed_s, sU_s;
            DevBuf<int> lastpos_s;
            bool lastpos_valid = false;
        } srt[2];
        int64_t lastpos_carried_epochs = 0;
        bool chain = true;
        bool defer_prep_w = false;
        bool prep_w_pending = false;
        bool prep_w_cm = false;
        bool cen_ready = false;
        bool cen_fresh = false;
        long sk_stride = 0;
        int res_every = 0;
        DevBuf<int> sk_keys, sk_keys2, sk_vals;
        DevBuf<int> sk_tmp;
        bool refine_on = true;
        int grid_mult = 2;
        bool scout_on = true;
        DevBuf<int> scout_g;
        DevBuf<float> tq;
        double share_forecast = 1.0;
        struct Cost {
            hipEvent_t ev[8] = {};
            bool have = false;
        } cost;
        struct Centroids { DevBuf<float> Cc, rg, csq, cmax2; DevBuf<char> Cst;
                           DevBuf<char> Cst_plain;
                           int n_slots = 0, n_cstages = 0, n_img_stages = 0; } cen[2];
        DevBuf<unsigned long long> need, need2;
        DevBuf<int> glist, gcnt;
        DevBuf<int> tlist, tcnt;
        DevBuf<int2> tile_counts;
        DevBuf<int> tile_ticket;
        bool fuse_select = true;
        int64_t sel_fused_passes = 0, sel_launched_passes = 0, sel_ticket_tiles = 0;
        DevBuf<int2> items;
        int item_slots = 0;
        int screen_slots = 0;
        bool item_queue = true;
        int item_len_pct = 125;
    } ex;
    int n_kchunks = 0;
    int n_ublocks = 0;
    bool tl_big = false;
    bool wide = false;
    int tl_bm = 128, tl_bn = 128, tl_xtile = 0, tl_wfrag = 0, tl_wtile = 0;
    int dp = 0;
    int stage_bytes = 0;
    int stage_units = 0;
    int nt = 1;
    bool swapped = false;
    int norm_p = 2;
    double norm_pr = 0.0;
    hipStream_t stream = nullptr;
    bool own_stream = false;

    DevBuf<float> W, wsq, SC, T, ACC, P1, P2;
    DevBuf<float> Ud;
    DevBuf<char> Wst;
    DevBuf<char> Wst_lo;
    DevBuf<char> Wfst;
    int fr_kg = 0, fr_stages = 0;
    DevBuf<char> Wfimg;
    DevBuf<char> ftX;
    int ft_kchunks = 0, ft_ublocks = 0;
    int n_stages = 0;
    bool w_dirty = true, wsq_dirty = true, wf_dirty = true, wp_dirty = true;
    bool wn_fresh = false;

    const float* Xd = nullptr;
    DevBuf<float> X_owned;
    long N = 0, Np = 0;
    DevBuf<int> bmu;
    bool bmu_valid = false;
    struct EarlyUpdate { bool armed = false, done = false; double sigma = 0, eta = 0; int neigh_f64 = 0; } early;
    DevBuf<unsigned long long> best64;
    int n_cus = 0;
    struct SegScratch {
        DevBuf<int> skey, srow;
        DevBuf<int> tmp;
        DevBuf<int> kA, kB;
        DevBuf<float> vA, vB;
        long cap = 0;
        DevBuf<int> cs_table;
        long cs_blocks = 0;
    };
    SegScratch seg;
    DevBuf<float> xsq;
    DevBuf<__bf16> Xb;
    DevBuf<float> xmax2;
    DevBuf<float> wn;
    DevBuf<float> wmax2;

    DevBuf<float> qX; DevBuf<int> qbmu, qbmu2; DevBuf<float> qxsq; DevBuf<__bf16> qXb;
    DevBuf<double> qX64;
    long qcap = 0;
    DevBuf<double> dsum;
    DevBuf<int> qe_list, qe_ids, qe_cnt; DevBuf<float> qe_X, qe_xsq;
    int64_t qe_rows = 0, qe_rows_sqrt = 0;
    struct Top2Scratch {
        bool on = true;
        DevBuf<float> m;
        DevBuf<int> excl;
        DevBuf<float> X, xsq;
        DevBuf<int> ids1, ids2;
        int64_t rows = 0, rows_f32 = 0;
    } t2;
    SegScratch st_seg;
    bool streaming = false;
    struct Slot {
        DevBuf<float> dX; DevBuf<__bf16> dXb; DevBuf<float> dxsq; DevBuf<int> dbmu;
        long cap = 0;
        hipEvent_t copied = nullptr, consumed = nullptr;
        bool used = false;
    } slot[2];
    hipStream_t copy_stream = nullptr;
    int slot_idx = 0;

    bool use_graph = false;
    bool capturing = false;
    hipGraphExec_t gexec = nullptr;
    unsigned long alloc_gen = 0, gexec_gen = 0;
    const void* gexec_rows = nullptr;
    long gexec_n = -1;
    int graph_warm = 0;
    DevBuf<NeighParams> np_dev;
    DevBuf<int2> bands;
    bool use_bands = true;

    int verify_rows = 0;
    bool verifying = false;
    DevBuf<int> vf_rows, vf_picks, vf_best, vf_bad;
    DevBuf<float> vf_X;
    int vf_cap = 0;
    int64_t verify_launches = 0, verify_rows_checked = 0;
    bool fuse_merge_prep = true;
    bool counting_sort = true;
    int env_bf16_parts = 0;
    int env_f32_parts = 0;
    bool debug = false;
    struct KernelSlots { const void* fn; size_t lds; int per_cu; };
    std::vector<KernelSlots> kernel_slots;
    int staged_blocks_done = -1;
    bool async_copies = false;
    int prof = 0;
    std::vector<EventPair> pending, pool;
    double ms[SOM_K_COUNT] = {0};
    int64_t launches[SOM_K_COUNT] = {0};

    std::string err;
};

namespace {

int fail(som_handle* h, const std::string& msg) {
    if (h) h->err = msg; else g_create_error = msg;
    return 1;
}
int fail_hip(som_handle* h, const char* what, hipError_t e) {
    return fail(h, std::string(what) + ": " + hipGetErrorString(e));
}

struct DeviceGuard {
    int prev = -1;
    bool moved = false;
    explicit DeviceGuard(const som_handle* h) {
        if (!h) return;
        if (hipGetDevice(&prev) != hipSuccess) prev = -1;
        if (prev != h->cfg.device) { (void)hipSetDevice(h->cfg.device); moved = true; }
    }
    ~DeviceGuard() { if (moved && prev >= 0) (void)hipSetDevice(prev); }
    DeviceGuard(const DeviceGuard&) = delete;
    DeviceGuard& operator=(const DeviceGuard&) = delete;
};

#define HIPCHK(h, call)                                              \
    do {                                                             \
        hipError_t e_ = (call);                                      \
        if (e_ != hipSuccess) return fail_hip((h), #call, e_);       \
    } while (0)

}

template <typename T>
int DevBuf<T>::alloc(som_handle* h, size_t n) {
    reset();
    if (n == 0) n = 1;
    if (h->capturing) return fail(h, "allocation during graph capture");
// ... 874 lines not shown
    int n = 0;
    if (hipGetDeviceCount(&n) != hipSuccess) return 0;
    return n;
}

const char* som_last_error(const som_handle* h) { return h ? h->err.c_str() : g_create_error.c_str(); }

int som_create(const som_config* cfg, som_handle** out) {
    if (!out) return fail(nullptr, "som_create: out is NULL");
    *out = nullptr;
    if (!cfg) return fail(nullptr, "som_create: cfg is NULL");
    if (cfg->x < 1 || cfg->y < 1 || cfg->input_len < 1) return fail(nullptr, "som_create: x, y, input_len must be >= 1");
    if ((long)cfg->x * cfg->y > (1L << 30)) return fail(nullptr, "som_create: map too large");
    if (cfg->distance < 0 || cfg->distance > SOM_DIST_NORM_P_NO_OPT) return fail(nullptr, "som_create: unknown distance id");
    if (cfg->norm_p < 0 || cfg->norm_p > PW_MAX_P) return fail(nullptr, "som_create: norm_p out of range (1..16)");
    if (cfg->norm_p_real != 0.0 && !(cfg->norm_p_real > 0.0 && cfg->norm_p_real <= 64.0))
        return fail(nullptr, "som_create: norm_p_real out of range (0 < p <= 64)");
    if (cfg->distance >= SOM_DIST_MANHATTAN && cfg->precision != SOM_PREC_F32 && cfg->precision != SOM_PREC_EXACT)
        return fail(nullptr, "som_create: manhattan / norm_p distances are float32 VALU kernels (precision f32)");
    if (cfg->neighborhood < 0 || cfg->neighborhood > SOM_NEIGH_TRIANGLE)
        return fail(nullptr, "som_create: unknown neighbourhood id");
    if (cfg->neighborhood == SOM_NEIGH_MEXICAN_HAT && cfg->compact_support && cfg->topology == SOM_TOPO_RECTANGULAR &&
        cfg->x != cfg->y)
        return fail(nullptr, "som_create: mexican_hat with compact_support needs a square map on the rectangular topology "
                             "(the reference's second mask on px does not broadcast otherwise, neighborhoods.py:70)");
    if (cfg->topology != SOM_TOPO_RECTANGULAR && cfg->topology != SOM_TOPO_HEXAGONAL)
        return fail(nullptr, "som_create: unknown topology id");
    if (cfg->topology == SOM_TOPO_HEXAGONAL && cfg->neighborhood == SOM_NEIGH_TRIANGLE)
        return fail(nullptr, "som_create: the hexagonal topology has no triangle neighbourhood (xpysom.py:271-279)");
    if (cfg->precision < SOM_PREC_F32 || cfg->precision > SOM_PREC_EXACT)
        return fail(nullptr, "som_create: unknown precision id");
    if (cfg->precision == SOM_PREC_RETIRED_2 || cfg->precision == SOM_PREC_RETIRED_4)
        return fail(nullptr, "som_create: the split-operand precisions (ids 2 and 4: 'bf16x3', 'f16x3') are retired -- "
                             "precision 'exact' returns float32's own BMUs, faster");
    if (cfg->precision != SOM_PREC_F32 && cfg->precision != SOM_PREC_EXACT) {
        if (cfg->distance == SOM_DIST_EUCLIDEAN_NO_OPT)
            return fail(nullptr, "som_create: bf16 precision implements 'euclidean' and 'cosine' "
                                 "('euclidean_no_opt' has the same argmin as 'euclidean')");
    }
    int ndev = 0;
    hipError_t e = hipGetDeviceCount(&ndev);
    if (e != hipSuccess || ndev < 1) return fail(nullptr, "som_create: no HIP device available");
    if (cfg->device < 0 || cfg->device >= ndev) return fail(nullptr, "som_create: device ordinal out of range");

    som_handle* h = new som_handle();
    h->cfg = *cfg;
    if (cfg->precision == SOM_PREC_EXACT) {
        if ((cfg->distance == SOM_DIST_EUCLIDEAN && cfg->input_len <= 128) ||
            ((cfg->distance == SOM_DIST_EUCLIDEAN || cfg->distance == SOM_DIST_COSINE) && cfg->input_len > 128)) h->exact = true;
        else h->cfg.precision = SOM_PREC_F32;
    }
    cfg = &h->cfg;
    h->X = cfg->x; h->Y = cfg->y; h->K = cfg->x * cfg->y; h->D = cfg->input_len;
    h->D1p = (int)round_up(h->D + 1, 4);
    h->norm_p = cfg->norm_p > 0 ? cfg->norm_p : 2;
    if (cfg->norm_p_real != 0.0 && (cfg->distance == SOM_DIST_NORM_P || cfg->distance == SOM_DIST_NORM_P_NO_OPT)) h->norm_pr = cfg->norm_p_real;
    h->ks32 = (int)cdiv(h->D, 32);
    h->f16 = cfg->precision == SOM_PREC_F16 || h->exact;
    h->tiled = (cfg->precision == SOM_PREC_BF16 || cfg->precision == SOM_PREC_F16 || h->exact) && h->D > 128;
    if (h->tiled) {
        h->tl_big = h->K >= 4096;
        if (h->tl_big) {
            using C = TileCfg<8, 2, 4>;
            h->tl_bm = C::BM; h->tl_bn = C::BN; h->tl_xtile = C::XTILE; h->tl_wfrag = C::WFRAG; h->tl_wtile = C::WTILE;
        } else {
            using C = TileCfg<4, 2, 2>;
            h->tl_bm = C::BM; h->tl_bn = C::BN; h->tl_xtile = C::XTILE; h->tl_wfrag = C::WFRAG; h->tl_wtile = C::WTILE;
        }
        h->n_kchunks = (int)cdiv((long)h->D, TL_BK);
        h->n_ublocks = (int)cdiv(h->K, h->tl_bn);
    }
    h->wide = h->tiled && h->tl_big && h->n_kchunks <= 25;
    if (const char* e = dev_env("SOM_BF16_WIDE")) if (std::atoi(e) == 0) h->wide = false;
    if (h->exact && h->tiled && !h->wide) {
        h->exact = false; h->f16 = false; h->tiled = false;
        h->cfg.precision = SOM_PREC_F32;
    }
    h->ex_patch = h->exact && h->K >= 2 * EX_GROUP;
    if (const char* e = dev_env("SOM_EXACT_PATCH")) if (std::atoi(e) == 0) h->ex_patch = false;
    h->dp = h->tiled ? TL_BK * h->n_kchunks : 32 * h->ks32;
    h->stage_bytes = h->wide ? wd_stage_bytes(h->n_kchunks) : k16_stage_bytes(h->ks32);
    h->stage_units = h->wide ? WD_STAGE_UNITS : K16_STAGE_UNITS;
    h->nt = cfg->neighborhood == SOM_NEIGH_MEXICAN_HAT ? (cfg->compact_support ? 4 : 2) : 1;
    h->swapped = cfg->neighborhood == SOM_NEIGH_MEXICAN_HAT && cfg->compact_support && cfg->topology == SOM_TOPO_RECTANGULAR;
    if (cfg->topology == SOM_TOPO_HEXAGONAL && cfg->neighborhood != SOM_NEIGH_BUBBLE) h->nt *= cfg->compact_support ? 4 : 3;
    int rc = 0;
    auto bail = [&](int code) { g_create_error = h->err; som_destroy(h); return code; };
    DeviceGuard dev_guard(h);
    {
        int cur = -1;
        if (hipGetDevice(&cur) != hipSuccess || cur != cfg->device) return bail(fail(h, "hipSetDevice failed"));
    }
    {
        hipDeviceProp_t prop;
        if (hipGetDeviceProperties(&prop, cfg->device) == hipSuccess) h->n_cus = prop.multiProcessorCount;
    }
    if (cfg->stream) { h->stream = (hipStream_t)cfg->stream; }
    else {
        if (hipStreamCreateWithFlags(&h->stream, hipStreamNonBlocking) != hipSuccess)
            return bail(fail(h, "hipStreamCreate failed"));
        h->own_stream = true;
    }
    const size_t KD1 = (size_t)h->K * h->D1p;
    if ((rc = h->W.alloc(h, (size_t)h->K * h->D))) return bail(rc);
    if ((rc = h->wsq.alloc(h, (size_t)h->K))) return bail(rc);
    if (h->ex_patch) {
        if ((rc = h->Wp.alloc(h, (size_t)h->K * h->D))) return bail(rc);
        if ((rc = h->wsq_p.alloc(h, (size_t)h->K))) return bail(rc);
        if ((rc = h->ex_perm.alloc(h, (size_t)h->K))) return bail(rc);
        if ((rc = h->ex_inv.alloc(h, (size_t)h->K))) return bail(rc);
        std::vector<int> perm;
        bool blocks = true;
        if (const char* e = dev_env("SOM_EXACT_SUB44")) blocks = std::atoi(e) != 0;
        h->ex_sub44 = blocks && patch_order_blocks(h->X, h->Y);
        patch_order(h->X, h->Y, perm, blocks);
        std::vector<int> inv((size_t)h->K);
        for (int p = 0; p < h->K; ++p) inv[(size_t)perm[(size_t)p]] = p;
        if (hipMemcpy(h->ex_perm, perm.data(), (size_t)h->K * sizeof(int), hipMemcpyHostToDevice) != hipSuccess ||
            hipMemcpy(h->ex_inv, inv.data(), (size_t)h->K * sizeof(int), hipMemcpyHostToDevice) != hipSuccess)
            return bail(fail(h, "hipMemcpy of the patch-order tables failed"));
    }
    if ((rc = h->SC.alloc(h, KD1 + (size_t)h->K))) return bail(rc);
    if ((rc = h->Ud.alloc(h, (size_t)h->nt * h->K))) return bail(rc);
    if ((rc = h->T.alloc(h, KD1 * h->nt))) return bail(rc);
    if ((rc = h->ACC.alloc(h, KD1))) return bail(rc);
    if ((rc = h->P1.alloc(h, (size_t)h->nt * h->Y * h->Y))) return bail(rc);
    if ((rc = h->P2.alloc(h, (size_t)h->X * h->nt * h->X))) return bail(rc);
    if ((rc = h->dsum.alloc(h, 1))) return bail(rc);
    {
        if ((rc = h->np_dev.alloc(h, 1))) return bail(rc);
        if (const char* e = std::getenv("SOM_GRAPH")) h->use_graph = std::atoi(e) != 0;
        if (const char* e = dev_env("SOM_BF16_PARTS")) h->env_bf16_parts = std::atoi(e);
        if (const char* e = dev_env("SOM_F32_PARTS")) h->env_f32_parts = std::atoi(e);
        h->debug = std::getenv("SOM_DEBUG") != nullptr;
        if (const char* e = std::getenv("SOM_VERIFY")) h->verify_rows = std::max(0, std::atoi(e));
        if (const char* e = dev_env("SOM_EXACT_PASS_ROWS")) h->ex.pass_rows_override = std::atol(e);
        if (const char* e = dev_env("SOM_EXACT_DEBUG_REFUSE_ABOVE")) h->ex.hook_refuse_above = std::atol(e);
        if (const char* e = dev_env("SOM_EXACT_PAIRS")) h->ex.hook_pairs = std::max(1L, std::atol(e));
        h->ex.hook_refuse_skip = dev_env("SOM_EXACT_DEBUG_REFUSE_SKIP") != nullptr;
        if (const char* e = dev_env("SOM_EXACT_TWO_ROUND")) h->ex.two_round = std::atoi(e) != 0 ? 1 : 0;
        if (const char* e = dev_env("SOM_EXACT_SEED")) h->ex.seed_on = std::atoi(e) != 0;
        if (const char* e = std::getenv("SOM_EXACT_SKIP")) h->ex.skip_mode = std::atoi(e);
        if (const char* e = std::getenv("SOM_EXACT_TOP2")) h->t2.on = std::atoi(e) != 0;
        if (const char* e = dev_env("SOM_EXACT_SUBBLOCKS")) h->ex.sub_blocks = std::atoi(e) != 0;
        if (const char* e = dev_env("SOM_EXACT_REFINE")) h->ex.refine_on = std::atoi(e) != 0;
        if (const char* e = dev_env("SOM_EXACT_QUEUE")) { h->ex.item_queue = std::atoi(e) != 0; if (std::atoi(e) >= 25) h->ex.item_len_pct = std::atoi(e); }
        if (const char* e = dev_env("SOM_EXACT_SCOUT")) h->ex.scout_on = std::atoi(e) != 0;
        if (const char* e = dev_env("SOM_EXACT_GRID_MULT")) h->ex.grid_mult = std::max(1, std::atoi(e));
        if (const char* e = dev_env("SOM_EXACT_RESORT")) h->ex.res_every = std::max(0, std::atoi(e));
        if (const char* e = dev_env("SOM_ASYNC_COPIES")) h->async_copies = std::atoi(e) != 0;
        if (const char* e = dev_env("SOM_FUSE_MERGE")) h->fuse_merge_prep = std::atoi(e) != 0;
        if (const char* e = dev_env("SOM_EXACT_CHAIN")) h->ex.chain = std::atoi(e) != 0;
        if (const char* e = dev_env("SOM_EXACT_FUSE_SELECT")) h->ex.fuse_select = std::atoi(e) != 0;
        if (const char* e = dev_env("SOM_COUNTING_SORT")) h->counting_sort = std::atoi(e) != 0;
        h->use_bands = h->X > 256 || h->Y > 256;
        if (const char* e = dev_env("SOM_NO_BANDS")) h->use_bands = std::atoi(e) == 0;
        const size_t nb = (size_t)h->nt * (cdiv(h->Y, LM_BM) + cdiv(h->X, LM_BM));
        if ((rc = h->bands.alloc(h, nb))) return bail(rc);
    }
    if (hipMemsetAsync(h->W, 0, (size_t)h->K * h->D * sizeof(float), h->stream) != hipSuccess ||
        hipMemsetAsync(h->T, 0, KD1 * h->nt * sizeof(float), h->stream) != hipSuccess ||
        hipMemsetAsync(h->ACC, 0, KD1 * sizeof(float), h->stream) != hipSuccess)
        return bail(fail(h, "hipMemsetAsync failed"));
    if (h->D > 128) {
        h->ft_kchunks = (int)cdiv(h->D, FT_BK);
        h->ft_ublocks = (int)cdiv(h->K, FT_BN);
        if ((rc = h->Wfimg.alloc(h, (size_t)h->ft_ublocks * h->ft_kchunks * FT_WTILE))) return bail(rc);
    }
    if (h->D <= 128) {
        int kg = 1;
        while (kg * 8 < h->D) kg *= 2;
        h->fr_kg = kg;
        h->fr_stages = (int)cdiv(h->K, FR_STAGE_UNITS);
        if ((rc = h->Wfst.alloc(h, (size_t)h->fr_stages * fr_stage_bytes(kg)))) return bail(rc);
    }
    if (h->cfg.precision != SOM_PREC_F32) {
        h->n_stages = (int)cdiv(h->K, h->stage_units);
        size_t bytes = (size_t)h->n_stages * h->stage_bytes;
        if (h->tiled && !h->wide) bytes = (size_t)h->n_ublocks * h->n_kchunks * h->tl_wtile;
        if ((rc = h->Wst.alloc(h, bytes))) return bail(rc);
        if (h->exact && !h->tiled) {
            if ((rc = h->Wst_lo.alloc(h, bytes))) return bail(rc);
            if (hipMemsetAsync(h->Wst_lo, 0, bytes, h->stream) != hipSuccess) return bail(fail(h, "hipMemsetAsync failed"));
        }
        if ((rc = h->xmax2.alloc(h, 2))) return bail(rc);
        if ((rc = h->wn.alloc(h, (size_t)h->K))) return bail(rc);
        if ((rc = h->wmax2.alloc(h, 2))) return bail(rc);
        if (hipMemsetAsync(h->Wst, 0, bytes, h->stream) != hipSuccess) return bail(fail(h, "hipMemsetAsync failed"));
    }
    if (hipStreamSynchronize(h->stream) != hipSuccess) return bail(fail(h, "hipStreamSynchronize failed"));
    *out = h;
    return 0;
}

void som_destroy(som_handle* h) {
    if (!h) return;
    DeviceGuard dev_guard(h);
    (void)som_comm_destroy(h);
    if (h->comm_stream) (void)hipStreamDestroy(h->comm_stream);
    if (h->ev_block) (void)hipEventDestroy(h->ev_block);
    if (h->ev_comm) (void)hipEventDestroy(h->ev_comm);
    if (h->stream) (void)hipStreamSynchronize(h->stream);
    if (h->gexec) (void)hipGraphExecDestroy(h->gexec);
    for (auto& ep : h->pending) { (void)hipEventDestroy(ep.a); (void)hipEventDestroy(ep.b); }
    for (auto& ep : h->pool) { (void)hipEventDestroy(ep.a); (void)hipEventDestroy(ep.b); }
    if (h->ex.cost.have) for (auto& e : h->ex.cost.ev) (void)hipEventDestroy(e);
    if (h->ex.fb_ready) (void)hipEventDestroy(h->ex.fb_ready);
    for (auto& sl : h->slot) {
        if (sl.copied) (void)hipEventDestroy(sl.copied);
        if (sl.consumed) (void)hipEventDestroy(sl.consumed);
    }
    if (h->ex.pass_host) (void)hipHostFree(h->ex.pass_host);
    if (h->copy_stream) (void)hipStreamDestroy(h->copy_stream);
    if (h->own_stream && h->stream) (void)hipStreamDestroy(h->stream);
    delete h;
}

int som_set_weights(som_handle* h, const float* w_host) {
    DeviceGuard dev_guard(h);
    if (!h || !w_host) return fail(h, "som_set_weights: NULL argument");
    if (h->f16 && !h->exact && h->cfg.distance != SOM_DIST_COSINE) {
        for (long k = 0; k < h->K; ++k) {
            double q = 0.0;
            for (int d = 0; d < h->D; ++d) { const double v = w_host[k * h->D + d]; q += v * v; }
            if (q > (double)HALF_MAX * HALF_MAX && q <= 1.0e300)
                return fail(h, "som_set_weights: precision 'f16' needs units of norm <= 65504 (float16 range): scale the data, or use 'bf16' / 'f32'");
        }
    }
    if (int rc = h2d_blocking(h, h->W, w_host, (size_t)h->K * h->D * sizeof(float))) return rc;
    HIPCHK(h, hipStreamSynchronize(h->stream));
    mark_codebook_changed(h);
    return 0;
}

int som_get_weights(som_handle* h, float* w_host) {
    DeviceGuard dev_guard(h);
    if (!h || !w_host) return fail(h, "som_get_weights: NULL argument");
    return d2h_blocking(h, w_host, h->W, (size_t)h->K * h->D * sizeof(float));
}

static int adopt_rows(som_handle* h, int64_t n_rows) {
    h->bmu.reset(); h->xsq.reset(); h->Xb.reset();
    h->bmu_valid = false;
    h->ex.plan.order_lost();
    h->ex.srt[0].lastpos_valid = false;
    h->seg = som_handle::SegScratch{};
    h->N = n_rows;
    h->Np = round_up(n_rows, ROW_PAD);
    if (n_rows > 0x7fffffffL) return fail(h, "som_set_data: more than 2^31-1 rows per GPU");
    if (int rc = h->bmu.alloc(h, (size_t)n_rows)) return rc;
    if (n_rows > 0)
        if (int rc = seg_reserve(h, h->seg, n_rows)) return rc;
    const bool bf_cos_tiled = h->cfg.precision != SOM_PREC_F32 && h->cfg.distance == SOM_DIST_COSINE && h->tiled;
    if (needs_xsq(h) || bf_cos_tiled) {
        if (int rc = h->xsq.alloc(h, (size_t)n_rows * (h->exact ? 2 : 1))) return rc;
        if (needs_xsq(h)) if (int rc = row_sq(h, h->Xd, n_rows, h->xsq)) return rc;
    }
    if (h->cfg.precision != SOM_PREC_F32 && n_rows > 0) {
        if (int rc = h->Xb.alloc(h, (size_t)h->Np * h->dp)) return rc;
        if (int rc = prep_rows_bf16(h, h->Xd, n_rows, h->Np, h->Xb, h->xmax2, h->xsq)) return rc;
    }
    HIPCHK(h, hipStreamSynchronize(h->stream));
    if (h->f16 && !h->exact && n_rows > 0) {
        float m2 = 0.0f;
        if (int rc = d2h_blocking(h, &m2, h->xmax2, sizeof(float))) return rc;
        if (!(m2 <= HALF_MAX * HALF_MAX))
            return fail(h, "som_set_data: precision 'f16' needs rows of norm <= 65504 (float16 range): scale the data, or use 'bf16' / 'f32'");
    }
    if (h->exact && n_rows > 0) {
        bool ok = exact_reserve(h, n_rows) == 0;
        if (ok && exact_skip_wanted(h) && !h->wide)
            ok = exact_skip_reserve(h, h->ex.srt[0], n_rows, h->ex.stride) == 0;
        if (!ok) { (void)hipGetLastError(); h->err.clear(); }
    }
    return 0;
}

int som_set_data(som_handle* h, const float* x_host, int64_t n_rows) {
    DeviceGuard dev_guard(h);
    if (!h || n_rows < 0 || (!x_host && n_rows > 0)) return fail(h, "som_set_data: bad argument");
    h->Xd = nullptr;
    if (int rc = h->X_owned.alloc(h, (size_t)n_rows * h->D)) return rc;
    if (n_rows > 0)
        if (int rc = h2d_blocking(h, h->X_owned, x_host, (size_t)n_rows * h->D * sizeof(float))) return rc;
    h->Xd = h->X_owned;
    return adopt_rows(h, n_rows);
}

int som_set_data_device(som_handle* h, const void* x_dev, int64_t n_rows) {
    DeviceGuard dev_guard(h);
    if (!h || n_rows < 0 || (!x_dev && n_rows > 0)) return fail(h, "som_set_data_device: bad argument");
    h->X_owned.reset();
    h->Xd = (const float*)x_dev;
    return adopt_rows(h, n_rows);
}

int som_sync_producer(som_handle* h, uint64_t stream, int32_t has_stream) {
    DeviceGuard dev_guard(h);
    if (!h) return 1;
    if (!has_stream) { HIPCHK(h, hipDeviceSynchronize()); return 0; }
    hipStream_t st = stream == 1 ? (hipStream_t)0 : stream == 2 ? hipStreamPerThread : (hipStream_t)(uintptr_t)stream;
    HIPCHK(h, hipStreamSynchronize(st));
    return 0;
}

int som_copy_to_host(som_handle* h, const void* x_dev, uint64_t bytes, void* dst_host) {
// ... 635 lines not shown
        size_t bytes = (size_t)h->n_stages * h->stage_bytes;
        if (h->tiled && !h->wide) bytes = (size_t)h->n_ublocks * h->n_kchunks * h->tl_wtile;
        HIPCHK(h, hipMemsetAsync(h->Wst, 0, bytes, h->stream));
    }
    if ((which & 2) && h->Wfst) HIPCHK(h, hipMemsetAsync(h->Wfst, 0, (size_t)h->fr_stages * fr_stage_bytes(h->fr_kg), h->stream));
    if ((which & 2) && h->Wfimg) HIPCHK(h, hipMemsetAsync(h->Wfimg, 0, (size_t)h->ft_ublocks * h->ft_kchunks * FT_WTILE, h->stream));
    return 0;
}

int som_debug_operand_crc(som_handle* h, int32_t which, uint64_t* out) {
    DeviceGuard dev_guard(h);
    if (!h || !out) return 1;
    uint64_t hash = 0xcbf29ce484222325ull;
    std::vector<unsigned char> host;
    auto add = [&](const void* dev, size_t bytes) -> int {
        if (dev == nullptr || bytes == 0) return 0;
        host.resize(bytes);
        if (int rc = d2h_blocking(h, host.data(), dev, bytes)) return rc;
        for (size_t i = 0; i < bytes; ++i) { hash ^= host[i]; hash *= 0x100000001b3ull; }
        return 0;
    };
    HIPCHK(h, hipStreamSynchronize(h->stream));
    const bool half = h->cfg.precision != SOM_PREC_F32;
    size_t st_bytes = (size_t)h->n_stages * h->stage_bytes;
    if (h->tiled && !h->wide) st_bytes = (size_t)h->n_ublocks * h->n_kchunks * h->tl_wtile;
    int rc = 0;
    switch (which) {
    case 0: rc = add(h->Wst, half ? st_bytes : 0); break;
    case 1: rc = add(h->Wst_lo, st_bytes); break;
    case 2:
        for (int st = 0; h->Wfst && st < h->fr_stages && rc == 0; ++st)
            rc = add((const char*)h->Wfst + (size_t)st * fr_stage_bytes(h->fr_kg), (size_t)FR_UT * h->fr_kg * 1024 + 64 * sizeof(float));
        break;
    case 3: rc = add(h->ex_patch ? (const float*)h->wsq_p : (const float*)h->wsq, (size_t)h->K * sizeof(float)); break;
    case 4: rc = add(h->wn, half ? (size_t)h->K * sizeof(float) : 0); break;
    case 5: rc = add(h->wmax2, half ? 2 * sizeof(float) : 0); break;
    case 6:
        if (h->ex.cen_ready)
            for (int lv = 0; lv < (h->wide ? 1 : 2) && rc == 0; ++lv) {
                auto& c = h->ex.cen[lv];
                if ((rc = add(c.Cc, (size_t)c.n_slots * h->D * sizeof(float)))) break;
                if ((rc = add(c.rg, (size_t)c.n_slots * sizeof(float)))) break;
                if ((rc = add(c.csq, (size_t)c.n_slots * sizeof(float)))) break;
                rc = add(c.cmax2, 2 * sizeof(float));
            }
        break;
    case 7: rc = add(h->ex_patch ? (const float*)h->Wp : (const float*)h->W, (size_t)h->K * h->D * sizeof(float)); break;
    default: return fail(h, "som_debug_operand_crc: unknown buffer");
    }
    if (rc) return rc;
    *out = hash;
    return 0;
}

int som_debug_exact_centroids(som_handle* h, int32_t level, float* C_out, float* r_out, float* csq_out, int32_t* n_slots_out) {
    DeviceGuard dev_guard(h);
    if (!h || !n_slots_out) return fail(h, "som_debug_exact_centroids: NULL argument");
    if (!h->ex.cen_ready) return fail(h, "som_debug_exact_centroids: the handle holds no centroids (no launch has planned yet)");
    if (level < 0 || level >= (h->wide ? 1 : 2)) return fail(h, "som_debug_exact_centroids: no such level");
    const auto& c = h->ex.cen[level];
    *n_slots_out = c.n_slots;
    HIPCHK(h, hipStreamSynchronize(h->stream));
    if (C_out) if (int rc = d2h_blocking(h, C_out, c.Cc, (size_t)c.n_slots * h->D * sizeof(float))) return rc;
    if (r_out) if (int rc = d2h_blocking(h, r_out, c.rg, (size_t)c.n_slots * sizeof(float))) return rc;
    if (csq_out) if (int rc = d2h_blocking(h, csq_out, c.csq, (size_t)c.n_slots * sizeof(float))) return rc;
    return 0;
}

int som_policy_eval(int32_t which, const double* costs, const double* args, int32_t* out) {
    if (!costs || !args || !out) return 1;
    policy::Costs c;
    c.full_total = costs[0]; c.full_screen = costs[1]; c.plan_total = costs[2]; c.plan_over = costs[3]; c.plan_over_scout = costs[4];
    c.blk_ms = costs[5]; c.l2_ms_group = costs[6]; c.l2_ratio = costs[7]; c.sort_ms = costs[8];
    switch (which) {
    case 0: *out = policy::commit_scouted_plan(c, args[0], args[1]); return 0;
    case 1: *out = policy::level2_from_sample(c, args[0], args[1], args[2]); return 0;
    case 2: *out = policy::level2_pays(c, args[0], args[1]); return 0;
    case 3: *out = policy::sort_paid(c, args[0], args[1], args[2], (int)args[3]); return 0;
    case 4: *out = policy::plan_idle(c, args[0]); return 0;
    case 5: *out = policy::scout_continues(c, args[0], args[1], args[2]); return 0;
    case 6: *out = policy::rows_worth_a_scout(args[0], args[1], args[2]); return 0;
    }
    return 1;
}

int som_policy_replay(int32_t n_launches, const double* script, double* out) {
    if (n_launches < 0 || !script || !out) return 1;
    policy::PlanState st;
    for (int32_t i = 0; i < n_launches; ++i) {
        const double* in = script + (size_t)i * SOM_POLICY_REPLAY_IN;
        double* o = out + (size_t)i * SOM_POLICY_REPLAY_OUT;
        policy::LaunchFacts f;
        f.resident = in[0] != 0.0; f.have_last = in[1] != 0.0; f.rows = (const void*)(uintptr_t)in[2]; f.n_rows = (long)in[3];
        f.can_skip = in[4] != 0.0; f.scout_ok = in[5] != 0.0; f.wide = in[6] != 0.0; f.wide_can = in[7] != 0.0; f.wide_scout_ok = in[8] != 0.0;
        f.l2_fits_lds = in[9] != 0.0; f.have_lo_image = in[10] != 0.0; f.blocks_per_row = in[11];
        f.skip_mode = (int)in[12]; f.refine_on = in[13] != 0.0; f.sub_blocks = in[14] != 0.0; f.res_every = (int)in[15];
        policy::LaunchPlan p = st.begin(f);
        const bool asked_rows = p.estimate;
        const bool row_no = asked_rows && st.rows_sampled(in[16], p);
        const bool asked_tiles = p.estimate && p.sample_tiles && in[17] >= 0.0;
        const bool tile_no = asked_tiles && st.tiles_sampled(in[17], in[18], f, p);
        policy::LaunchOutcome oc;
        oc.t_total = in[19]; oc.t_screen = in[20]; oc.t_l2 = in[21]; oc.t_sort = in[22];
        oc.screen_timed = p.time_phases; oc.l2_timed = p.time_phases && p.skip && p.level2; oc.sort_timed = p.time_phases && p.skip && p.resort;
        oc.blocks_total = (int64_t)in[24];
        oc.blocks_run = p.skip ? (int64_t)in[23] : oc.blocks_total;
        oc.groups_run = p.skip ? (int64_t)in[25] : oc.blocks_total / policy::TILES_PER_GROUP;
        oc.pairs_in = (int64_t)in[26]; oc.pairs_out = p.refine ? (int64_t)in[27] : 0; oc.scout_wins = (p.skip && p.scout && f.have_last) ? (int64_t)in[28] : 0;
        st.end(f, p, oc);
        o[0] = p.skip; o[1] = p.resort; o[2] = p.scout; o[3] = p.level2; o[4] = p.estimate; o[5] = p.sample_tiles; o[6] = p.refine; o[7] = p.time_phases;
        o[8] = asked_rows; o[9] = asked_tiles; o[10] = row_no; o[11] = tile_no;
        for (int k = 0; k < 2; ++k) {
            const policy::Pause& ps = st.pause(k == 0);
            o[12 + 3 * k] = ps.cooldown; o[13 + 3 * k] = ps.idle; o[14 + 3 * k] = ps.pause;
        }
    }
    return 0;
}

int som_debug_mfma16(som_handle* h, const uint16_t* a_host, const uint16_t* b_host, const float* c_host, float* d_host,
                     int32_t is_f16) {
    DeviceGuard dev_guard(h);
    if (!h || !a_host || !b_host || !c_host || !d_host) return fail(h, "som_debug_mfma16: NULL argument");
    DevBuf<uint16_t> a, b;
    DevBuf<float> c, d;
    int rc = 0;
    if ((rc = a.alloc(h, 512)) || (rc = b.alloc(h, 512)) || (rc = c.alloc(h, 256)) || (rc = d.alloc(h, 256))) return rc;
    if (h2d_blocking(h, a, a_host, 1024) || h2d_blocking(h, b, b_host, 1024) || h2d_blocking(h, c, c_host, 1024)) return 1;
    if (is_f16) debug_mfma16_kernel<F16><<<dim3(1), dim3(64), 0, h->stream>>>(a, b, c, d);
    else debug_mfma16_kernel<Bf16><<<dim3(1), dim3(64), 0, h->stream>>>(a, b, c, d);
    return d2h_blocking(h, d_host, d, 1024);
}

int som_debug_device_bytes(int64_t* out) {
    if (!out) return 1;
    *out = g_dev_bytes.load();
    return 0;
}

int som_debug_exact_chain_stats(som_handle* h, int64_t* carried_epochs) {
    if (!h || !carried_epochs) return fail(h, "som_debug_exact_chain_stats: NULL argument");
    *carried_epochs = h->ex.lastpos_carried_epochs;
    return 0;
}

int som_debug_exact_select_stats(som_handle* h, int64_t* fused_passes, int64_t* launched_passes, int64_t* ticket_tiles) {
    if (!h || !fused_passes || !launched_passes || !ticket_tiles) return fail(h, "som_debug_exact_select_stats: NULL argument");
    *fused_passes = h->ex.sel_fused_passes;
    *launched_passes = h->ex.sel_launched_passes;
    *ticket_tiles = h->ex.sel_ticket_tiles;
    return 0;
}

int som_debug_qe_stats(som_handle* h, int64_t* rows, int64_t* rows_sqrt) {
    if (!h || !rows || !rows_sqrt) return fail(h, "som_debug_qe_stats: NULL argument");
    *rows = h->qe_rows;
    *rows_sqrt = h->qe_rows_sqrt;
    return 0;
}

int som_debug_stamps(som_handle* h, int64_t n_pairs, uint64_t* out_host) {
    DeviceGuard dev_guard(h);
    if (!h) return 1;
#ifdef SOM_STAMPS
    static unsigned long long* buf = nullptr;
    static int64_t cap = 0;
    HIPCHK(h, hipStreamSynchronize(h->stream));
    if (out_host) {
        if (n_pairs > cap) return fail(h, "som_debug_stamps: more pairs than the buffer holds");
        HIPCHK(h, hipMemcpy(out_host, buf, (size_t)n_pairs * 16, hipMemcpyDeviceToHost));
        return 0;
    }
    if (buf) { (void)hipFree(buf); buf = nullptr; cap = 0; }
    if (n_pairs > 0) {
        HIPCHK(h, hipMalloc((void**)&buf, (size_t)n_pairs * 16));
        HIPCHK(h, hipMemset(buf, 0, (size_t)n_pairs * 16));
        cap = n_pairs;
    }
    HIPCHK(h, hipMemcpyToSymbol(HIP_SYMBOL(g_som_stamps), &buf, sizeof(buf)));
    return 0;
#else
    (void)n_pairs; (void)out_host;
    return fail(h, "som_debug_stamps: this library was built without -DSOM_STAMPS (tools/stamps.py builds the diagnostic one)");
#endif
}

int som_patch_order(int32_t x, int32_t y, int32_t* perm_out) {
    if (x <= 0 || y <= 0 || !perm_out || (int64_t)x * y > 0x7fffffffLL) return 1;
    std::vector<int> perm;
    patch_order(x, y, perm);
    std::copy(perm.begin(), perm.end(), perm_out);
    return 0;
}

int som_exact_stats(som_handle* h, int64_t* rows, int64_t* rows_fallback, int64_t* passes) {
    if (!h) return 1;
    if (rows) *rows = h->ex.rows_total;
    if (rows_fallback) *rows_fallback = h->ex.rows_fallback;
    if (passes) *passes = h->ex.chunks;
    return 0;
}

int som_exact_top2_stats(som_handle* h, int64_t* rows, int64_t* rows_f32) {
    if (!h || !rows || !rows_f32) return fail(h, "som_exact_top2_stats: NULL argument");
    *rows = h->t2.rows; *rows_f32 = h->t2.rows_f32;
    return 0;
}

int som_exact_skip_stats(som_handle* h, int64_t* blocks_run, int64_t* blocks_total) {
    if (!h || !blocks_run || !blocks_total) return 1;
    *blocks_run = h->ex.blocks_run; *blocks_total = h->ex.blocks_total;
    return 0;
}

int som_exact_resident_stats(som_handle* h, int64_t* planned_epochs, int64_t* sorts) {
    if (!h || !planned_epochs || !sorts) return 1;
    *planned_epochs = h->ex.plan.stats().planned; *sorts = h->ex.plan.stats().resorts;
    return 0;
}

int som_exact_scout_stats(som_handle* h, int64_t* scouted_launches, int64_t* transient_planned) {
    if (!h || !scouted_launches || !transient_planned) return 1;
    *scouted_launches = h->ex.plan.stats().scouted; *transient_planned = h->ex.plan.stats().tr_planned;
    return 0;
}

int som_exact_refine_stats(som_handle* h, int64_t* pairs_in, int64_t* pairs_out) {
    if (!h || !pairs_in || !pairs_out) return 1;
    *pairs_in = h->ex.plan.stats().pairs_refined_in; *pairs_out = h->ex.plan.stats().pairs_refined_out;
    return 0;
}

int som_exact_last_counts(som_handle* h, int32_t* counts_out, int64_t n) {
    DeviceGuard dev_guard(h);
    if (!h || !counts_out || n < 0) return fail(h, "som_exact_last_counts: bad argument");
    if (!h->exact || n > h->ex.stride) return fail(h, "som_exact_last_counts: no screen pass of that many rows");
    if (int rc = d2h_blocking(h, counts_out, h->ex.rowcnt, (size_t)n * sizeof(int32_t))) return rc;
    return 0;
}

int som_sync(som_handle* h) {
    DeviceGuard dev_guard(h);
    if (!h) return 1;
    HIPCHK(h, hipStreamSynchronize(h->stream));
    return 0;
}

int som_profile_enable(som_handle* h, int32_t on) {
    DeviceGuard dev_guard(h);
    if (!h) return 1;
    if (!on) if (int rc = resolve_profile(h)) return rc;
    h->prof = on == 2 ? 2 : on != 0;
    return 0;
}

int som_profile_get(som_handle* h, int32_t kernel, double* total_ms, int64_t* launches) {
    DeviceGuard dev_guard(h);
    if (!h || kernel < 0 || kernel >= SOM_K_COUNT) return fail(h, "som_profile_get: bad argument");
    if (int rc = resolve_profile(h)) return rc;
    if (total_ms) *total_ms = h->ms[kernel];
    if (launches) *launches = h->launches[kernel];
    return 0;
}

int som_profile_reset(som_handle* h) {
    DeviceGuard dev_guard(h);
    if (!h) return 1;
    if (int rc = resolve_profile(h)) return rc;
    for (int i = 0; i < SOM_K_COUNT; ++i) { h->ms[i] = 0; h->launches[i] = 0; }
    return 0;
}

}
```

### xpysom_dask_amd/engine.py

```python
import ctypes as C

import numpy as np

from . import _lib


class SomHipError(RuntimeError):
    pass


def _f32(a):
    return np.ascontiguousarray(a, dtype=np.float32)


class HipEngine:
    def __init__(self, x, y, input_len, *, distance="euclidean", neighborhood="gaussian",
                 std_coeff=0.5, compact_support=False, precision="exact", device=0, stream=None,
                 topology="rectangular", norm_p=0, norm_p_real=0.0):
        self._lib = _lib.load()
        self._h = None
        self.K, self.D = int(x) * int(y), int(input_len)
        self.x, self.y = int(x), int(y)
        self.n_rows = 0
        self._keepalive = None
# ... 133 lines not shown
        arr = np.frombuffer(buf, dtype=np.float32, count=n).reshape(shape)
        weakref.finalize(buf, self._lib.som_pinned_free, p)
        return arr

    def stream_epoch_accumulate(self, chunks, sigma, eta, neigh_f64):
        self._check(self._lib.som_stream_begin(self._h))
        for chunk in chunks:
            chunk = _f32(chunk)
            if chunk.ndim != 2 or chunk.shape[1] != self.D:
                raise ValueError("chunk must be (n, %d), got %r" % (self.D, chunk.shape))
            self._check(self._lib.som_stream_rows(self._h, self._fp(chunk), chunk.shape[0]))
        self._check(self._lib.som_stream_end(self._h, float(sigma), float(eta), int(bool(neigh_f64))))
        self.sync()

    def epoch_fetch(self, want_bmu=True):
        num = np.empty((self.K, self.D), dtype=np.float32)
        den = np.empty((self.K,), dtype=np.float32)
        bmu = np.empty((self.n_rows,), dtype=np.int32) if want_bmu else None
        self._check(self._lib.som_epoch_fetch(self._h, self._fp(num), self._fp(den),
                                              self._ip(bmu) if want_bmu else None))
        return num, den, bmu

    def accum_device_ptr(self):
        p, n = C.c_void_p(), C.c_int64()
        self._check(self._lib.som_accum_device_ptr(self._h, C.byref(p), C.byref(n)))
        return p.value, n.value

    def stream_ptr(self):
        p = C.c_void_p()
        self._check(self._lib.som_get_stream(self._h, C.byref(p)))
        return int(p.value or 0)

    def accum_tensor(self):
        import torch
        ptr, n = self.accum_device_ptr()

        class _Alias:
            __cuda_array_interface__ = {"shape": (n,), "typestr": "<f4", "data": (ptr, False),
                                        "version": 2, "strides": None}
        return torch.as_tensor(_Alias(), device=torch.device("cuda", self.device))

    def bmu(self, x, quantization=False):
        x = _f32(x)
        if x.ndim != 2 or x.shape[1] != self.D:
            raise ValueError("x must be (n, %d), got %r" % (self.D, x.shape))
        ids = np.empty((x.shape[0],), dtype=np.int32)
        mode = _lib.SOM_BMU_QUANTIZATION if quantization else _lib.SOM_BMU_ACTIVATION
        self._check(self._lib.som_bmu(self._h, self._fp(x), x.shape[0], mode, self._ip(ids)))
        return ids

    def bmu_device(self, dev_ptr, n_rows, quantization=False):
        ids = np.empty((int(n_rows),), dtype=np.int32)
        mode = _lib.SOM_BMU_QUANTIZATION if quantization else _lib.SOM_BMU_ACTIVATION
        self._check(self._lib.som_bmu_device(self._h, C.c_void_p(dev_ptr), int(n_rows), mode, self._ip(ids)))
        return ids

    def quantization_error_device(self, dev_ptr, n_rows):
        out = C.c_double()
        self._check(self._lib.som_quantization_error_device(self._h, C.c_void_p(dev_ptr), int(n_rows), C.byref(out)))
        return out.value

    def bmu_f64(self, x):
        x = np.ascontiguousarray(x, dtype=np.float64)
        if x.ndim != 2 or x.shape[1] != self.D:
            raise ValueError("x must be (n, %d), got %r" % (self.D, x.shape))
        ids = np.empty((x.shape[0],), dtype=np.int32)
        self._check(self._lib.som_bmu_f64(self._h, x.ctypes.data_as(C.POINTER(C.c_double)), x.shape[0], self._ip(ids)))
        return ids

    def bmu_top2(self, x):
        x = _f32(x)
        if x.ndim != 2 or x.shape[1] != self.D:
            raise ValueError("x must be (n, %d), got %r" % (self.D, x.shape))
        a = np.empty((x.shape[0],), dtype=np.int32)
        b = np.empty((x.shape[0],), dtype=np.int32)
        self._check(self._lib.som_bmu_top2(self._h, self._fp(x), x.shape[0], self._ip(a), self._ip(b)))
        return a, b

    def bmu_top2_device(self, dev_ptr, n_rows):
        a = np.empty((int(n_rows),), dtype=np.int32)
        b = np.empty((int(n_rows),), dtype=np.int32)
        self._check(self._lib.som_bmu_top2_device(self._h, C.c_void_p(dev_ptr), int(n_rows), self._ip(a), self._ip(b)))
        return a, b

    def distance_matrix(self, x, quantization=False):
        x = _f32(x)
        if x.ndim != 2 or x.shape[1] != self.D:
            raise ValueError("x must be (n, %d), got %r" % (self.D, x.shape))
        out = np.empty((x.shape[0], self.K), dtype=np.float32)
        mode = _lib.SOM_BMU_QUANTIZATION if quantization else _lib.SOM_BMU_ACTIVATION
        self._check(self._lib.som_distance_matrix(self._h, self._fp(x), x.shape[0], mode, self._fp(out)))
        return out

    def quantization_error(self, x):
        x = _f32(x)
        out = C.c_double()
        self._check(self._lib.som_quantization_error(self._h, self._fp(x), x.shape[0], C.byref(out)))
        return out.value

    def set_verify(self, n_rows):
        self._check(self._lib.som_set_verify(self._h, int(n_rows)))

    def verify_stats(self):
        a, b = C.c_int64(), C.c_int64()
        self._check(self._lib.som_verify_stats(self._h, C.byref(a), C.byref(b)))
        return a.value, b.value

    def debug_corrupt_operands(self, which=3):
        self._check(self._lib.som_debug_corrupt_operands(self._h, int(which)))

    def debug_exact_centroids(self, level):
        n = C.c_int32()
        self._check(self._lib.som_debug_exact_centroids(self._h, int(level), None, None, None, C.byref(n)))
        cen = np.empty((n.value, self.D), dtype=np.float32)
        rad = np.empty((n.value,), dtype=np.float32)
        csq = np.empty((n.value,), dtype=np.float32)
        self._check(self._lib.som_debug_exact_centroids(self._h, int(level), self._fp(cen), self._fp(rad), self._fp(csq), C.byref(n)))
        return cen, rad, csq

    def debug_mfma16(self, a, b, c, f16=True):
        a = np.ascontiguousarray(a).view(np.uint16).reshape(16, 32)
        b = np.ascontiguousarray(b).view(np.uint16).reshape(32, 16)
        c = np.ascontiguousarray(c, dtype=np.float32).reshape(16, 16)
        d = np.empty((16, 16), dtype=np.float32)
        self._check(self._lib.som_debug_mfma16(self._h, a.ctypes.data_as(C.c_void_p), b.ctypes.data_as(C.c_void_p),
                                               self._fp(c), self._fp(d), int(bool(f16))))
        return d

    def exact_stats(self):
        a, b, c = C.c_int64(), C.c_int64(), C.c_int64()
        self._check(self._lib.som_exact_stats(self._h, C.byref(a), C.byref(b), C.byref(c)))
        return a.value, b.value, c.value

    def qe_stats(self):
        a, b = C.c_int64(), C.c_int64()
        self._check(self._lib.som_debug_qe_stats(self._h, C.byref(a), C.byref(b)))
        return a.value, b.value

    def exact_top2_stats(self):
        a, b = C.c_int64(), C.c_int64()
        self._check(self._lib.som_exact_top2_stats(self._h, C.byref(a), C.byref(b)))
        return a.value, b.value

    def exact_chain_stats(self):
        a = C.c_int64()
        self._check(self._lib.som_debug_exact_chain_stats(self._h, C.byref(a)))
        return a.value

    def exact_select_stats(self):
        a, b, c = C.c_int64(), C.c_int64(), C.c_int64()
        self._check(self._lib.som_debug_exact_select_stats(self._h, C.byref(a), C.byref(b), C.byref(c)))
        return a.value, b.value, c.value

    def exact_skip_stats(self):
        a, b = C.c_int64(), C.c_int64()
        self._check(self._lib.som_exact_skip_stats(self._h, C.byref(a), C.byref(b)))
        return a.value, b.value

    def exact_resident_stats(self):
        a, b = C.c_int64(), C.c_int64()
        self._check(self._lib.som_exact_resident_stats(self._h, C.byref(a), C.byref(b)))
        return a.value, b.value

    def exact_scout_stats(self):
        a, b = C.c_int64(), C.c_int64()
        self._check(self._lib.som_exact_scout_stats(self._h, C.byref(a), C.byref(b)))
        return a.value, b.value

    def exact_refine_stats(self):
        a, b = C.c_int64(), C.c_int64()
        self._check(self._lib.som_exact_refine_stats(self._h, C.byref(a), C.byref(b)))
        return a.value, b.value

    def exact_last_counts(self, n):
        out = np.empty((int(n),), dtype=np.int32)
        self._check(self._lib.som_exact_last_counts(self._h, self._ip(out), int(n)))
        return out

    def sync(self):
        self._check(self._lib.som_sync(self._h))

    def profile_enable(self, on=True):
        self._check(self._lib.som_profile_enable(self._h, 2 if on == "bmu" else int(bool(on))))

    def profile_reset(self):
        self._check(self._lib.som_profile_reset(self._h))

    def profile_get(self, kernel):
        ms, n = C.c_double(), C.c_int64()
        self._check(self._lib.som_profile_get(self._h, _lib.SOM_KERNELS[kernel], C.byref(ms), C.byref(n)))
        return ms.value, n.value
```

Before: 535.5 million.

## Fuse exact skip-plan level1, level2 and list building into one kernel

Adds a fused plan kernel that computes per-row seeds and thresholds, walks level-1 centroid stages, builds the level-2 active list in LDS, walks level 2, and emits the tile/group lists in a single launch. It replaces the separate plan, memset and list kernels when the chain is on, level 2 is active, the plan grid is one partition and the LDS fits. The aim is to cut launch overhead and global round-trips of the need masks. The cost is higher LDS and register pressure, plus a single partition per tile that may lower parallelism. It also adds debug counters and an environment knob for the partition cap.

```diff
diff --git a/xpysom_dask_amd/_lib.py b/xpysom_dask_amd/_lib.py
--- a/xpysom_dask_amd/_lib.py
+++ b/xpysom_dask_amd/_lib.py
@@ -78,6 +78,8 @@
     "som_debug_qe_stats": (C.c_int, [_H, C.POINTER(C.c_int64), C.POINTER(C.c_int64)]),
     "som_debug_exact_chain_stats": (C.c_int, [_H, C.POINTER(C.c_int64)]),
     "som_debug_exact_select_stats": (C.c_int, [_H, C.POINTER(C.c_int64), C.POINTER(C.c_int64), C.POINTER(C.c_int64)]),
+    "som_debug_exact_plan_stats": (C.c_int, [_H, C.POINTER(C.c_int64), C.POINTER(C.c_int64)]),
+    "som_debug_exact_last_plan": (C.c_int, [_H, C.POINTER(C.c_int32)]),
     "som_policy_eval": (C.c_int, [C.c_int32, C.POINTER(C.c_double), C.POINTER(C.c_double), C.POINTER(C.c_int32)]),
     "som_policy_replay": (C.c_int, [C.c_int32, C.POINTER(C.c_double), C.POINTER(C.c_double)]),
     "som_patch_order": (C.c_int, [C.c_int32, C.c_int32, _I]),
diff --git a/xpysom_dask_amd/csrc/exact_host.hpp b/xpysom_dask_amd/csrc/exact_host.hpp
--- a/xpysom_dask_amd/csrc/exact_host.hpp
+++ b/xpysom_dask_amd/csrc/exact_host.hpp
@@ -420,6 +420,7 @@
                                                                   n_items, n_items + 1, ex.item_len_pct);
 }
 
+template <int KS32, class E> constexpr bool plan_fused_fits() { return !(KS32 == 4 && std::is_same<E, Bf16>::value); }
 template <class E>
 int exact_skip_plan(som_handle* h, som_handle::ExactScratch::SortedRows& sr, long s0, long n, const float* xmax2, const ExactBound& eb,
                     const int* lastpos2, bool time_l2 = false) {
@@ -431,12 +432,39 @@
     const auto& c0 = ex.cen[0];
     const auto& c1 = ex.cen[1];
     const long want = (1024 + tiles - 1) / tiles;
-    const dim3 pgrid((unsigned)tiles, (unsigned)std::max<long>(1, std::min<long>({want, 4L, (long)c0.n_cstages})));
+    const long parts_cap = ex.hook_plan_parts > 0 ? ex.hook_plan_parts : 4L;
+    const dim3 pgrid((unsigned)tiles, (unsigned)std::max<long>(1, std::min<long>({want, parts_cap, (long)c0.n_cstages})));
     const size_t lds1 = 2 * (size_t)h->stage_bytes + (size_t)c0.n_cstages * 8;
     const size_t lds2 = 2 * (size_t)h->stage_bytes + (size_t)c0.n_cstages * 64 * sizeof(int) + (size_t)c1.n_cstages * 8;
     const bool l2 = ex.lp.level2;
     const int force = ex.skip_mode == 3 ? 1 : 0;
     const __bf16* Xs = sr.Xb_s + s0 * h->dp;
+    const size_t lds = lds2 + (size_t)c0.n_cstages * 8 + (size_t)SK_TILE * sizeof(float);
+    const bool fits = h->ks32 != 4 || plan_fused_fits<4, E>();
+    if (ex.fuse_plan && ex.chain && l2 && lastpos2 == nullptr && pgrid.y == 1 && !time_l2 && lds <= 160 * 1024 && fits) {
+        PlanListsOut lo;
+        lo.n_groups = (int)cdiv(h->K, EX_GROUP);
+        lo.glist = ex.glist; lo.gcnt = ex.gcnt; lo.tile_counts = ex.tile_counts; lo.tlist = ex.tlist; lo.tcnt = ex.tcnt;
+        lo.tile_ticket = ex.tile_ticket;
+        lo.done = &ctr->lists_done; lo.blocks_run = &ctr->blocks_run; lo.groups_run = &ctr->groups_run;
+        lo.slots = ex.item_queue ? (ex.screen_slots > 0 ? ex.screen_slots : ex.item_slots) : 0;
+        lo.items = ex.item_queue ? ex.items + 8 : nullptr;
+        lo.n_items = (int*)ex.items.p; lo.item_ctr = lo.n_items + 1; lo.len_pct = ex.item_len_pct;
+#define SOM_PLAN_FUSED_CASE(k) case k: if constexpr (plan_fused_fits<k, E>()) { \
+        { int pc; if (int rc = kernel_per_cu(h, (const void*)exact_plan_fused_kernel<k, E>, 64 * K16_NW, lds, &pc)) return rc; } \
+        exact_plan_fused_kernel<k, E><<<dim3((unsigned)tiles), block, lds, h->stream>>>(Xs, n, c0.Cst, c0.n_cstages, c0.cmax2, c1.Cst, c1.n_slots, \
+            c1.cmax2, sr.xsq_s + s0, sr.xerr_s + s0, xmax2, h->wmax2, h->wmax2 + 1, eb, sr.lastpos_s + s0, h->Wst, sr.seed_s + s0, force, lo); \
+        } break;
+        switch (h->ks32) {
+        SOM_PLAN_FUSED_CASE(1) SOM_PLAN_FUSED_CASE(2) SOM_PLAN_FUSED_CASE(3) SOM_PLAN_FUSED_CASE(4)
+        default: return fail(h, "exact: block skipping supports input_len <= 128");
+        }
+#undef SOM_PLAN_FUSED_CASE
+        ++ex.plan_fused_launches;
+        HIPCHK(h, hipGetLastError());
+        return 0;
+    }
+    ++ex.plan_split_launches;
     unsigned long long* const need2_clear = l2 && ex.chain ? ex.need2.p : nullptr;
     if (l2 && !ex.chain) HIPCHK(h, hipMemsetAsync(ex.need2, 0, (size_t)tiles * c1.n_cstages * sizeof(unsigned long long), h->stream));
 #define SOM_PLAN_CASE(k) case k: { \
diff --git a/xpysom_dask_amd/csrc/exact_skip.hpp b/xpysom_dask_amd/csrc/exact_skip.hpp
--- a/xpysom_dask_amd/csrc/exact_skip.hpp
+++ b/xpysom_dask_amd/csrc/exact_skip.hpp
@@ -332,6 +332,252 @@
     else prep_wsqh_body(blockIdx.x - w_blocks - c_blocks, wn, K, wmax2, xmax2, Wst, n_stages, k16_stage_bytes(KS32), stage_units, best64, n_rows, 1);
 }
 
+template <int KS32, class EL>
+__device__ __forceinline__ float plan_row_seed(const typename V8<typename EL::T>::t (&xrow)[KS32], long row, float q, float xe,
+                                               const ExactBound& eb, const ExactScales& sw, const char* __restrict__ Wst,
+                                               const int* __restrict__ lastpos, const int* __restrict__ lastpos2,
+                                               int* __restrict__ scout_wins, float* __restrict__ seed_s, int force_all) {
+    using bf16x8 = typename V8<typename EL::T>::t;
+    constexpr int STAGE = k16_stage_bytes(KS32);
+    const int lane = threadIdx.x & 63, quad = lane >> 4;
+    auto value_of = [&](int pos) -> float {
+        const char* stg = Wst + (long)(pos >> 6) * STAGE;
+        const int t16 = (pos >> 4) & 3, c = pos & 15;
+        float d = 0.0f;
+#pragma unroll
+        for (int ks = 0; ks < KS32; ++ks) {
+            const bf16x8 a = *(const bf16x8*)(stg + ((t16 * KS32 + ks) * 64 + quad * 16 + c) * 16);
+#pragma unroll
+            for (int jj = 0; jj < 8; ++jj) d = __builtin_fmaf((float)a[jj], (float)xrow[ks][jj], d);
+        }
+        d += __shfl_xor(d, 16, 64);
+        d += __shfl_xor(d, 32, 64);
+        return *(const float*)(stg + K16_T * KS32 * 1024 + (t16 * 16 + c) * 4) + d;
+    };
+    float vu = value_of(lastpos[row]);
+    if (lastpos2 != nullptr) {
+        const float v2 = value_of(lastpos2[row]);
+        const float Sq = sw.sx * sw.sw;
+        const float ua = q + 2.0f * (vu / Sq - sw.big), ub = q + 2.0f * (v2 / Sq - sw.big);
+        const bool win = ua < 0.9f * ub;
+        const unsigned long long wm = __ballot(win && quad == 0);
+        if (scout_wins != nullptr && lane == __builtin_ctzll(__ballot(true)) && wm != 0ull) atomicAdd(scout_wins, (int)__popcll(wm));
+        vu = (v2 < vu || !(vu == vu)) ? v2 : vu;
+    }
+    const float Sw = sw.sx * sw.sw;
+    const float e = ex_row_bound(eb, sw, q, xe);
+    const float f32s = ex_f32_share(eb, sw, q);
+    const float e_valu = 48.0f * 0x1p-24f * Sw * sw.bmag;
+    const float sd = vu + (e - f32s) * (1.0f + 1.0f / 1024.0f) + e_valu + Sw * sw.bmag * 0x1p-21f;
+    if (quad == 0) seed_s[row] = (sd > 0.0f && sd < 3.0e38f) ? sd : __builtin_inff();
+    const float e_one = 0.5f * (e - f32s) * (1.0f + 1.0f / 1024.0f) + e_valu;
+    const float tau_up = 2.0f * (((vu + e_one) - Sw * sw.big) / Sw) + 0x1p-20f * (sw.big + __builtin_fabsf(vu) / Sw);
+    const float xn = __builtin_sqrtf(q) * (1.0f + 1.0f / 1024.0f);
+    const float share = 2.0f * (eb.cA * xn * sw.wm + eb.cW * sw.wm * sw.wm);
+    const float U0 = q * (1.0f + 1.0f / 1024.0f) + tau_up + share * (1.0f + 1.0f / 1024.0f) + 0x1p-18f * (q + __builtin_fabsf(tau_up));
+    const float U = U0 < 0.0f ? 0.0f : U0;
+    float su = __builtin_sqrtf(U) * (1.0f + 1.0f / 1024.0f);
+    if (force_all || !(su == su) || !(su < 3.0e38f) || !(e == e)) su = __builtin_inff();
+    return su;
+}
+
+template <int KS32>
+__device__ __forceinline__ void plan_row_threshold(const ExactBound& eb, const ExactScales& sc, bool in_pass, float q, float xe, float su,
+                                                   float& P, float& bx) {
+    const float S = sc.sx * sc.sw;
+    float A = -__builtin_inff(), sU = 0.0f;
+    if (in_pass) {
+        const float ec = 0.5f * ex_row_bound(eb, sc, q, xe) * (1.0f + 1.0f / 1024.0f);
+        sU = su;
+        A = S * sc.big + ec - 0.5f * S * q * (1.0f - 1.0f / 1024.0f) + 0x1p-12f * S * (sc.big + q) + 0x1p-16f * S * sc.wm * sc.wm;
+        if (!(A == A) || !(A < 3.0e38f) || !(su < 3.0e38f)) {
+            A = __builtin_inff(); sU = 0.0f;
+        }
+    }
+    bx = up_to_half(sc.sx * sU * (1.0f + 1.0f / 1024.0f));
+    P = A + 0.5f * S * (1.0f + 1.0f / 1024.0f) * sU * sU * (1.0f + 0x1p-20f) + (float)(24 * (KS32 + 1)) * 0x1p-23f * S * sc.bmag;
+    if (!(bx < 3.0e38f) || !(P == P)) P = __builtin_inff();
+    if (A == -__builtin_inff()) P = -__builtin_inff();
+}
+template <class EL>
+__device__ __forceinline__ typename V8<typename EL::T>::t plan_extra_step(float bx) {
+    using E = typename EL::T;
+    typename V8<E>::t v;
+#pragma unroll
+    for (int jj = 0; jj < 8; ++jj) v[jj] = (E)0.0f;
+    if (((threadIdx.x & 63) >> 4) == 0 && bx < 3.0e38f) v[0] = (E)bx;
+    return v;
+}
+
+template <int KS32, class EL>
+__device__ __forceinline__ void plan_run_tile(int j, const typename V8<typename EL::T>::t (&a)[KS32], const f32x4& wv, float rneg,
+                                              const typename V8<typename EL::T>::t (&xf)[K16_SB][KS32],
+                                              const typename V8<typename EL::T>::t (&xe)[K16_SB], const float (&P)[K16_SB],
+                                              uint32_t& lane_bits) {
+    using E = typename EL::T;
+    using bf16x8 = typename V8<E>::t;
+    bf16x8 ae;
+#pragma unroll
+    for (int jj = 0; jj < 8; ++jj) ae[jj] = (E)0.0f;
+    if (((threadIdx.x & 63) >> 4) == 0) ae[0] = (E)rneg;
+    f32x4 acc[K16_SB];
+#pragma unroll
+    for (int sb = 0; sb < K16_SB; ++sb) acc[sb] = wv;
+#pragma unroll
+    for (int ks = 0; ks < KS32; ++ks)
+#pragma unroll
+        for (int sb = 0; sb < K16_SB; ++sb) acc[sb] = mfma16(a[ks], xf[sb][ks], acc[sb]);
+#pragma unroll
+    for (int sb = 0; sb < K16_SB; ++sb) acc[sb] = mfma16(ae, xe[sb], acc[sb]);
+#pragma unroll
+    for (int r = 0; r < 4; ++r) {
+        bool nd = false;
+#pragma unroll
+        for (int sb = 0; sb < K16_SB; ++sb) nd = nd || !(acc[sb][r] > P[sb]);
+        lane_bits |= nd ? (1u << (4 * j + r)) : 0u;
+    }
+}
+template <int KS32, class EL>
+__device__ __forceinline__ void plan_load_tile(const char* st, int t, typename V8<typename EL::T>::t (&a)[KS32], f32x4& wv, float& rneg) {
+    using bf16x8 = typename V8<typename EL::T>::t;
+    const int lane = threadIdx.x & 63;
+    const float* wq = (const float*)(st + K16_T * KS32 * 1024);
+#pragma unroll
+    for (int ks = 0; ks < KS32; ++ks) a[ks] = *(const bf16x8*)(st + ((t * KS32 + ks) * 64 + lane) * 16);
+    wv = *(const f32x4*)(wq + t * 16 + 4 * (lane >> 4));
+    rneg = wq[64 + t * 16 + (lane & 15)];
+}
+
+template <int KS32, class EL>
+__device__ __forceinline__ void plan_walk_level1(const char* __restrict__ Cst, int s_begin, int s_end, char* smem, unsigned long long* nl,
+                                                 const typename V8<typename EL::T>::t (&xf)[K16_SB][KS32],
+                                                 const typename V8<typename EL::T>::t (&xe)[K16_SB], const float (&P)[K16_SB]) {
+    using bf16x8 = typename V8<typename EL::T>::t;
+    constexpr int STAGE = k16_stage_bytes(KS32);
+    constexpr int PIECES = K16_T * KS32 + 1;
+    const int lane = threadIdx.x & 63, quad = lane >> 4, col = lane & 15;
+    const int wave = __builtin_amdgcn_readfirstlane(threadIdx.x >> 6);
+    auto dma_stage = [&](int s, char* dst) {
+        const char* src = Cst + (long)s * STAGE;
+        for (int p = wave; p < PIECES; p += K16_NW) lds_dma_16(src + (long)p * 1024 + lane * 16, dst + p * 1024);
+    };
+    if (s_begin < s_end) dma_stage(s_begin, smem);
+    for (int i = s_begin; i < s_end; ++i) {
+        asm volatile("s_waitcnt vmcnt(0) lgkmcnt(0)" ::: "memory");
+        __builtin_amdgcn_s_barrier();
+        asm volatile("" ::: "memory");
+        if (i + 1 < s_end) dma_stage(i + 1, smem + ((i + 1 - s_begin) & 1) * STAGE);
+        const char* st = smem + ((i - s_begin) & 1) * STAGE;
+        uint32_t lane_bits = 0u;
+        bf16x8 aA[KS32], aB[KS32];
+        f32x4 wvA, wvB;
+        float rnA, rnB;
+        plan_load_tile<KS32, EL>(st, 0, aA, wvA, rnA);
+        plan_load_tile<KS32, EL>(st, 1, aB, wvB, rnB);
+        plan_run_tile<KS32, EL>(0, aA, wvA, rnA, xf, xe, P, lane_bits);
+        plan_load_tile<KS32, EL>(st, 2, aA, wvA, rnA);
+        plan_run_tile<KS32, EL>(1, aB, wvB, rnB, xf, xe, P, lane_bits);
+        plan_load_tile<KS32, EL>(st, 3, aB, wvB, rnB);
+        plan_run_tile<KS32, EL>(2, aA, wvA, rnA, xf, xe, P, lane_bits);
+        plan_run_tile<KS32, EL>(3, aB, wvB, rnB, xf, xe, P, lane_bits);
+        const uint32_t any_row = row16_or(lane_bits);
+        if (col == 0 && any_row != 0u) {
+            const uint32_t lo = ((any_row & 15u) | (((any_row >> 4) & 15u) << 16)) << (4 * quad);
+            const uint32_t hi = (((any_row >> 8) & 15u) | (((any_row >> 12) & 15u) << 16)) << (4 * quad);
+            atomicOr(nl + (i - s_begin), ((unsigned long long)hi << 32) | lo);
+        }
+    }
+}
+
+__device__ __forceinline__ void plan_level2_list(const unsigned long long* need1, int n_cstages1, int n_slots2, int* act, int* act_n) {
+    const int lane = threadIdx.x & 63;
+    int cnt = 0;
+    for (int s1 = 0; s1 < n_cstages1; ++s1) {
+        const unsigned long long w = need1[s1];
+        const int g = s1 * 64 + lane;
+        const bool on = ((w >> lane) & 1ull) && 4 * (g >> 2) * 4 < n_slots2;
+        const unsigned long long mk = __ballot(on);
+        if (on) act[cnt + __popcll(mk & ((1ull << lane) - 1ull))] = g;
+        cnt += __popcll(mk);
+    }
+    if (lane == 0) *act_n = cnt;
+}
+
+template <int KS32, class EL>
+__device__ __forceinline__ void plan_walk_level2(const char* __restrict__ Cst, const int* act, int b0, int e0, char* smem,
+                                                 unsigned long long* nl, const typename V8<typename EL::T>::t (&xf)[K16_SB][KS32],
+                                                 const typename V8<typename EL::T>::t (&xe)[K16_SB], const float (&P)[K16_SB]) {
+    using bf16x8 = typename V8<typename EL::T>::t;
+    constexpr int STAGE = k16_stage_bytes(KS32);
+    static_assert(K16_NW == 4, "a wave per tile fills the slot's tail");
+    const int lane = threadIdx.x & 63, quad = lane >> 4, col = lane & 15;
+    const int wave = __builtin_amdgcn_readfirstlane(threadIdx.x >> 6);
+    constexpr int TQ = K16_T * KS32 * 1024;
+    auto frag_of = [&](int g, int sub, int ks, int q) -> const char* {
+        return Cst + (long)(g >> 4) * STAGE + (((((g >> 2) & 3) * KS32 + ks) * 64 + q * 16 + 4 * (g & 3) + sub) * 16);
+    };
+    auto dma_chunk = [&](int c0, char* dst) {
+        for (int p = wave; p < K16_T * KS32; p += K16_NW) {
+            const int j = p / KS32, ks = p - j * KS32;
+            if (c0 + 4 * j < e0) {
+                const int gi = c0 + 4 * j + (col >> 2);
+                const int g = gi < e0 ? act[gi] : act[c0 + 4 * j];
+                lds_dma_16(frag_of(g, col & 3, ks, quad), dst + p * 1024);
+            }
+        }
+    };
+    auto load_tail = [&](int c0) -> float {
+        const int i = lane & 15, gi = c0 + 4 * wave + (i >> 2);
+        if (lane >= 32 || gi >= e0) return lane < 16 ? __builtin_inff() : 0.0f;
+        const int g = act[gi];
+        return *(const float*)(Cst + (long)(g >> 4) * STAGE + TQ + (((lane >> 4) * 64) + ((g >> 2) & 3) * 16 + 4 * (g & 3) + (i & 3)) * 4);
+    };
+    auto store_tail = [&](char* dst, float v) {
+        if (lane < 32) *(float*)(dst + TQ + (((lane >> 4) * 64) + wave * 16 + (lane & 15)) * 4) = v;
+    };
+    if (b0 < e0) { dma_chunk(b0, smem); store_tail(smem, load_tail(b0)); }
+    int k = 0;
+    for (int c0 = b0; c0 < e0; c0 += 16, ++k) {
+        asm volatile("s_waitcnt vmcnt(0) lgkmcnt(0)" ::: "memory");
+        __builtin_amdgcn_s_barrier();
+        asm volatile("" ::: "memory");
+        char* sn = smem + ((k + 1) & 1) * STAGE;
+        float tail_n = 0.0f;
+        if (c0 + 16 < e0) { dma_chunk(c0 + 16, sn); tail_n = load_tail(c0 + 16); }
+        const char* st = smem + (k & 1) * STAGE;
+        uint32_t lane_bits = 0u;
+        bf16x8 aA[KS32], aB[KS32];
+        f32x4 wvA, wvB;
+        float rnA, rnB;
+        const bool h1 = c0 + 4 < e0, h2 = c0 + 8 < e0, h3 = c0 + 12 < e0;
+        plan_load_tile<KS32, EL>(st, 0, aA, wvA, rnA);
+        if (h1) plan_load_tile<KS32, EL>(st, 1, aB, wvB, rnB);
+        plan_run_tile<KS32, EL>(0, aA, wvA, rnA, xf, xe, P, lane_bits);
+        if (h1) {
+            if (h2) plan_load_tile<KS32, EL>(st, 2, aA, wvA, rnA);
+            plan_run_tile<KS32, EL>(1, aB, wvB, rnB, xf, xe, P, lane_bits);
+            if (h2) {
+                if (h3) plan_load_tile<KS32, EL>(st, 3, aB, wvB, rnB);
+                plan_run_tile<KS32, EL>(2, aA, wvA, rnA, xf, xe, P, lane_bits);
+                if (h3) plan_run_tile<KS32, EL>(3, aB, wvB, rnB, xf, xe, P, lane_bits);
+            }
+        }
+        const uint32_t any_row = row16_or(lane_bits);
+        if (col == 0 && any_row != 0u) {
+#pragma unroll
+            for (int j = 0; j < 4; ++j) {
+                const uint32_t nib = (any_row >> (4 * j)) & 15u;
+                const int gi = c0 + 4 * j + quad;
+                if (nib != 0u && gi < e0) {
+                    const int g = act[gi];
+                    atomicOr(nl + (g >> 4), (unsigned long long)nib << (4 * (g & 15)));
+                }
+            }
+        }
+        if (c0 + 16 < e0) store_tail(sn, tail_n);
+    }
+}
+
 template <int KS32, class EL, bool LEVEL2>
 __global__ __launch_bounds__(64 * K16_NW, LEVEL2 ? 3 : 2) void exact_plan_kernel(const __bf16* __restrict__ Xb, long N,
                                                                     const char* __restrict__ Cst, int n_cstages,
@@ -347,11 +593,9 @@
                                                                     int force_all, const int* __restrict__ lastpos2 = nullptr,
                                                                     int* __restrict__ scout_wins = nullptr,
                                                                     unsigned long long* __restrict__ need2_clear = nullptr) {
-    using E = typename EL::T;
-    using bf16x8 = typename V8<E>::t;
+    using bf16x8 = typename V8<typename EL::T>::t;
     constexpr int DP = 32 * KS32;
     constexpr int STAGE = k16_stage_bytes(KS32);
-    constexpr int PIECES = K16_T * KS32 + 1;
     extern __shared__ __attribute__((aligned(16))) char smem[];
     __shared__ int act_n;
 
@@ -362,279 +606,48 @@
 
     bf16x8 xf[K16_SB][KS32];
     bf16x8 xe[K16_SB];
-    float A[K16_SB], sU[K16_SB], P[K16_SB];
+    float P[K16_SB];
     const ExactScales sc = ex_scales(xmax2, cmax2, cmax2 + 1);
     const ExactScales sw = ex_scales(xmax2, wmax2, werr2);
-    const float S = sc.sx * sc.sw;
 #pragma unroll
     for (int sb = 0; sb < K16_SB; ++sb) {
         const long row = wave_s0 + sb * 16 + col;
 #pragma unroll
         for (int ks = 0; ks < KS32; ++ks) xf[sb][ks] = *(const bf16x8*)(Xb + row * DP + ks * 32 + quad * 8);
-        A[sb] = -__builtin_inff(); sU[sb] = 0.0f;
+        float q = 0.0f, xer = 0.0f, su = 0.0f;
         if (row < N) {
-            const float q = xsq[row], xe = xerr[row];
-            float su;
-            if (!LEVEL2) {
-                auto value_of = [&](int pos) -> float {
-                    const char* stg = Wst + (long)(pos >> 6) * STAGE;
-                    const int t16 = (pos >> 4) & 3, c = pos & 15;
-                    float d = 0.0f;
-#pragma unroll
-                    for (int ks = 0; ks < KS32; ++ks) {
-                        const bf16x8 a = *(const bf16x8*)(stg + ((t16 * KS32 + ks) * 64 + quad * 16 + c) * 16);
-#pragma unroll
-                        for (int jj = 0; jj < 8; ++jj) d = __builtin_fmaf((float)a[jj], (float)xf[sb][ks][jj], d);
-                    }
-                    d += __shfl_xor(d, 16, 64);
-                    d += __shfl_xor(d, 32, 64);
-                    return *(const float*)(stg + K16_T * KS32 * 1024 + (t16 * 16 + c) * 4) + d;
-                };
-                float vu = value_of(lastpos[row]);
-                if (lastpos2 != nullptr) {
-                    const float v2 = value_of(lastpos2[row]);
-                    const float Sq = sw.sx * sw.sw;
-                    const float ua = q + 2.0f * (vu / Sq - sw.big), ub = q + 2.0f * (v2 / Sq - sw.big);
-                    const bool win = ua < 0.9f * ub;
-                    const unsigned long long wm = __ballot(win && quad == 0);
-                    if (scout_wins != nullptr && lane == __builtin_ctzll(__ballot(true)) && wm != 0ull) atomicAdd(scout_wins, (int)__popcll(wm));
-                    vu = (v2 < vu || !(vu == vu)) ? v2 : vu;
-                }
-                const float Sw = sw.sx * sw.sw;
-                const float e = ex_row_bound(eb, sw, q, xe);
-                const float f32s = ex_f32_share(eb, sw, q);
-                const float e_valu = 48.0f * 0x1p-24f * Sw * sw.bmag;
-                const float sd = vu + (e - f32s) * (1.0f + 1.0f / 1024.0f) + e_valu + Sw * sw.bmag * 0x1p-21f;
-                if (quad == 0) seed_s[row] = (sd > 0.0f && sd < 3.0e38f) ? sd : __builtin_inff();
-                const float e_one = 0.5f * (e - f32s) * (1.0f + 1.0f / 1024.0f) + e_valu;
-                const float tau_up = 2.0f * (((vu + e_one) - Sw * sw.big) / Sw) + 0x1p-20f * (sw.big + __builtin_fabsf(vu) / Sw);
-                const float xn = __builtin_sqrtf(q) * (1.0f + 1.0f / 1024.0f);
-                const float share = 2.0f * (eb.cA * xn * sw.wm + eb.cW * sw.wm * sw.wm);
-                const float U0 = q * (1.0f + 1.0f / 1024.0f) + tau_up + share * (1.0f + 1.0f / 1024.0f) + 0x1p-18f * (q + __builtin_fabsf(tau_up));
-                const float U = U0 < 0.0f ? 0.0f : U0;
-                su = __builtin_sqrtf(U) * (1.0f + 1.0f / 1024.0f);
-                if (force_all || !(su == su) || !(su < 3.0e38f) || !(e == e)) su = __builtin_inff();
+            q = xsq[row]; xer = xerr[row];
+            if constexpr (!LEVEL2) {
+                su = plan_row_seed<KS32, EL>(xf[sb], row, q, xer, eb, sw, Wst, lastpos, lastpos2, scout_wins, seed_s, force_all);
                 if (quad == 0) sU_s[row] = su;
             } else {
                 su = sU_s[row];
             }
-            const float ec = 0.5f * ex_row_bound(eb, sc, q, xe) * (1.0f + 1.0f / 1024.0f);
-            sU[sb] = su;
-            A[sb] = S * sc.big + ec - 0.5f * S * q * (1.0f - 1.0f / 1024.0f) + 0x1p-12f * S * (sc.big + q) + 0x1p-16f * S * sc.wm * sc.wm;
-            if (!(A[sb] == A[sb]) || !(A[sb] < 3.0e38f) || !(su < 3.0e38f)) {
-                A[sb] = __builtin_inff(); sU[sb] = 0.0f;
-            }
-        }
-        const float bx = up_to_half(sc.sx * sU[sb] * (1.0f + 1.0f / 1024.0f));
-        P[sb] = A[sb] + 0.5f * S * (1.0f + 1.0f / 1024.0f) * sU[sb] * sU[sb] * (1.0f + 0x1p-20f) + (float)(24 * (KS32 + 1)) * 0x1p-23f * S * sc.bmag;
-        if (!(bx < 3.0e38f) || !(P[sb] == P[sb])) P[sb] = __builtin_inff();
-        if (A[sb] == -__builtin_inff()) P[sb] = -__builtin_inff();
-#pragma unroll
-        for (int jj = 0; jj < 8; ++jj) xe[sb][jj] = (E)0.0f;
-        if (quad == 0 && bx < 3.0e38f) xe[sb][0] = (E)bx;
+        }
+        float bx;
+        plan_row_threshold<KS32>(eb, sc, row < N, q, xer, su, P[sb], bx);
+        xe[sb] = plan_extra_step<EL>(bx);
     }
 
     int* act = (int*)(smem + 2 * STAGE);
     unsigned long long* nl = (unsigned long long*)(smem + 2 * STAGE + (LEVEL2 ? (size_t)n_cstages1 * 64 * sizeof(int) : 0));
     for (int i = tid; i < n_cstages; i += 64 * K16_NW) nl[i] = 0ull;
     if constexpr (LEVEL2) {
-        static_assert(K16_NW == 4, "a wave per tile fills the slot's tail");
-        if (wave == 0) {
-            int cnt = 0;
-            for (int s1 = 0; s1 < n_cstages1; ++s1) {
-                const unsigned long long w = need1[(long)blockIdx.x * n_cstages1 + s1];
-                const int g = s1 * 64 + lane;
-                const bool on = ((w >> lane) & 1ull) && 4 * (g >> 2) * 4 < n_slots;
-                const unsigned long long mk = __ballot(on);
-                if (on) act[cnt + __popcll(mk & ((1ull << lane) - 1ull))] = g;
-                cnt += __popcll(mk);
-            }
-            if (lane == 0) act_n = cnt;
-        }
+        if (wave == 0) plan_level2_list(need1 + (long)blockIdx.x * n_cstages1, n_cstages1, n_slots, act, &act_n);
         __syncthreads();
         const int n_act = act_n;
         const int c_all = (n_act + 15) / 16;
         const int b0 = 16 * (int)((long)c_all * blockIdx.y / gridDim.y);
         const int e0 = min(n_act, 16 * (int)((long)c_all * (blockIdx.y + 1) / gridDim.y));
-        constexpr int TQ = K16_T * KS32 * 1024;
-        auto frag_of = [&](int g, int sub, int ks, int q) -> const char* {
-            return Cst + (long)(g >> 4) * STAGE + (((((g >> 2) & 3) * KS32 + ks) * 64 + q * 16 + 4 * (g & 3) + sub) * 16);
-        };
-        auto dma_chunk = [&](int c0, char* dst) {
-            for (int p = wave; p < K16_T * KS32; p += K16_NW) {
-                const int j = p / KS32, ks = p - j * KS32;
-                if (c0 + 4 * j < e0) {
-                    const int gi = c0 + 4 * j + (col >> 2);
-                    const int g = gi < e0 ? act[gi] : act[c0 + 4 * j];
-                    lds_dma_16(frag_of(g, col & 3, ks, quad), dst + p * 1024);
-                }
-            }
-        };
-        auto load_tail = [&](int c0) -> float {
-            const int i = lane & 15, gi = c0 + 4 * wave + (i >> 2);
-            if (lane >= 32 || gi >= e0) return lane < 16 ? __builtin_inff() : 0.0f;
-            const int g = act[gi];
-            return *(const float*)(Cst + (long)(g >> 4) * STAGE + TQ + (((lane >> 4) * 64) + ((g >> 2) & 3) * 16 + 4 * (g & 3) + (i & 3)) * 4);
-        };
-        auto store_tail = [&](char* dst, float v) {
-            if (lane < 32) *(float*)(dst + TQ + (((lane >> 4) * 64) + wave * 16 + (lane & 15)) * 4) = v;
-        };
-        if (b0 < e0) { dma_chunk(b0, smem); store_tail(smem, load_tail(b0)); }
-        int k = 0;
-        for (int c0 = b0; c0 < e0; c0 += 16, ++k) {
-            asm volatile("s_waitcnt vmcnt(0) lgkmcnt(0)" ::: "memory");
-            __builtin_amdgcn_s_barrier();
-            asm volatile("" ::: "memory");
-            char* sn = smem + ((k + 1) & 1) * STAGE;
-            float tail_n = 0.0f;
-            if (c0 + 16 < e0) { dma_chunk(c0 + 16, sn); tail_n = load_tail(c0 + 16); }
-            const char* st = smem + (k & 1) * STAGE;
-            const float* wq = (const float*)(st + TQ);
-            auto load_tile = [&](int j, bf16x8 (&a)[KS32], f32x4& wv, float& rneg) {
-#pragma unroll
-                for (int ks = 0; ks < KS32; ++ks) a[ks] = *(const bf16x8*)(st + ((j * KS32 + ks) * 64 + lane) * 16);
-                wv = *(const f32x4*)(wq + j * 16 + 4 * quad);
-                rneg = wq[64 + j * 16 + col];
-            };
-            uint32_t lane_bits = 0u;
-            auto run_tile = [&](int j, const bf16x8 (&a)[KS32], const f32x4& wv, float rneg) {
-                bf16x8 ae;
-#pragma unroll
-                for (int jj = 0; jj < 8; ++jj) ae[jj] = (E)0.0f;
-                if (quad == 0) ae[0] = (E)rneg;
-                f32x4 acc[K16_SB];
-#pragma unroll
-                for (int sb = 0; sb < K16_SB; ++sb) acc[sb] = wv;
-#pragma unroll
-                for (int ks = 0; ks < KS32; ++ks)
-#pragma unroll
-                    for (int sb = 0; sb < K16_SB; ++sb) acc[sb] = mfma16(a[ks], xf[sb][ks], acc[sb]);
-#pragma unroll
-                for (int sb = 0; sb < K16_SB; ++sb) acc[sb] = mfma16(ae, xe[sb], acc[sb]);
-#pragma unroll
-                for (int r = 0; r < 4; ++r) {
-                    bool nd = false;
-#pragma unroll
-                    for (int sb = 0; sb < K16_SB; ++sb) nd = nd || !(acc[sb][r] > P[sb]);
-                    lane_bits |= nd ? (1u << (4 * j + r)) : 0u;
-                }
-            };
-            bf16x8 aA[KS32], aB[KS32];
-            f32x4 wvA, wvB;
-            float rnA, rnB;
-            const bool h1 = c0 + 4 < e0, h2 = c0 + 8 < e0, h3 = c0 + 12 < e0;
-            load_tile(0, aA, wvA, rnA);
-            if (h1) load_tile(1, aB, wvB, rnB);
-            run_tile(0, aA, wvA, rnA);
-            if (h1) {
-                if (h2) load_tile(2, aA, wvA, rnA);
-                run_tile(1, aB, wvB, rnB);
-                if (h2) {
-                    if (h3) load_tile(3, aB, wvB, rnB);
-                    run_tile(2, aA, wvA, rnA);
-                    if (h3) run_tile(3, aB, wvB, rnB);
-                }
-            }
-            const uint32_t any_row = row16_or(lane_bits);
-            if (col == 0 && any_row != 0u) {
-#pragma unroll
-                for (int j = 0; j < 4; ++j) {
-                    const uint32_t nib = (any_row >> (4 * j)) & 15u;
-                    const int gi = c0 + 4 * j + quad;
-                    if (nib != 0u && gi < e0) {
-                        const int g = act[gi];
-                        atomicOr(nl + (g >> 4), (unsigned long long)nib << (4 * (g & 15)));
-                    }
-                }
-            }
-            if (c0 + 16 < e0) store_tail(sn, tail_n);
-        }
+        plan_walk_level2<KS32, EL>(Cst, act, b0, e0, smem, nl, xf, xe, P);
         __syncthreads();
         for (int i = tid; i < n_cstages; i += 64 * K16_NW)
             if (nl[i] != 0ull) atomicOr(need + (long)blockIdx.x * n_cstages + i, nl[i]);
         return;
     }
-    const int n_walk = n_cstages;
-    const int s_begin = (int)((long)n_walk * blockIdx.y / gridDim.y);
-    const int s_end = (int)((long)n_walk * (blockIdx.y + 1) / gridDim.y);
-    auto item_of = [&](int i) -> int { return (i << 4) | 15; };
-    auto dma_stage = [&](int s, uint32_t tm, char* dst) {
-        const char* src = Cst + (long)s * STAGE;
-        for (int p = wave; p < PIECES; p += K16_NW)
-            if (p == PIECES - 1 || ((tm >> (p / KS32)) & 1u)) lds_dma_16(src + (long)p * 1024 + lane * 16, dst + p * 1024);
-    };
-    int st_cur = 0, st_next = 0;
-    uint32_t tm_cur = 0, tm_next = 0;
-    if (s_begin < s_end) {
-        const int it = item_of(s_begin);
-        st_cur = it >> 4; tm_cur = (uint32_t)it & 15u;
-        dma_stage(st_cur, tm_cur, smem);
-    }
-    for (int i = s_begin; i < s_end; ++i) {
-        asm volatile("s_waitcnt vmcnt(0) lgkmcnt(0)" ::: "memory");
-        __builtin_amdgcn_s_barrier();
-        asm volatile("" ::: "memory");
-        if (i + 1 < s_end) {
-            const int it = item_of(i + 1);
-            st_next = it >> 4; tm_next = (uint32_t)it & 15u;
-            dma_stage(st_next, tm_next, smem + ((i + 1 - s_begin) & 1) * STAGE);
-        }
-        const char* st = smem + ((i - s_begin) & 1) * STAGE;
-        const float* wq = (const float*)(st + K16_T * KS32 * 1024);
-        uint32_t lane_bits = 0u;
-        auto load_tile = [&](int t, bf16x8 (&a)[KS32], f32x4& wv, float& rneg) {
-#pragma unroll
-            for (int ks = 0; ks < KS32; ++ks) a[ks] = *(const bf16x8*)(st + ((t * KS32 + ks) * 64 + lane) * 16);
-            wv = *(const f32x4*)(wq + t * 16 + 4 * quad);
-            rneg = wq[64 + t * 16 + col];
-        };
-        auto run_tile = [&](int t16, const bf16x8 (&a)[KS32], const f32x4& wv, float rneg) {
-            bf16x8 ae;
-#pragma unroll
-            for (int jj = 0; jj < 8; ++jj) ae[jj] = (E)0.0f;
-            if (quad == 0) ae[0] = (E)rneg;
-            f32x4 acc[K16_SB];
-#pragma unroll
-            for (int sb = 0; sb < K16_SB; ++sb) acc[sb] = wv;
-#pragma unroll
-            for (int ks = 0; ks < KS32; ++ks)
-#pragma unroll
-                for (int sb = 0; sb < K16_SB; ++sb) acc[sb] = mfma16(a[ks], xf[sb][ks], acc[sb]);
-#pragma unroll
-            for (int sb = 0; sb < K16_SB; ++sb) acc[sb] = mfma16(ae, xe[sb], acc[sb]);
-#pragma unroll
-            for (int r = 0; r < 4; ++r) {
-                bool nd = false;
-#pragma unroll
-                for (int sb = 0; sb < K16_SB; ++sb) nd = nd || !(acc[sb][r] > P[sb]);
-                lane_bits |= nd ? (1u << (4 * t16 + r)) : 0u;
-            }
-        };
-        const uint32_t m0 = 15u, m1 = m0 & (m0 - 1u), m2 = m1 & (m1 - 1u), m3 = m2 & (m2 - 1u);
-        const int t0 = __builtin_ctz(m0), t1 = m1 ? __builtin_ctz(m1) : -1, t2 = m2 ? __builtin_ctz(m2) : -1, t3 = m3 ? __builtin_ctz(m3) : -1;
-        bf16x8 aA[KS32], aB[KS32];
-        f32x4 wvA, wvB;
-        float rnA, rnB;
-        load_tile(t0, aA, wvA, rnA);
-        if (t1 >= 0) load_tile(t1, aB, wvB, rnB);
-        run_tile(t0, aA, wvA, rnA);
-        if (t1 >= 0) {
-            if (t2 >= 0) load_tile(t2, aA, wvA, rnA);
-            run_tile(t1, aB, wvB, rnB);
-            if (t2 >= 0) {
-                if (t3 >= 0) load_tile(t3, aB, wvB, rnB);
-                run_tile(t2, aA, wvA, rnA);
-                if (t3 >= 0) run_tile(t3, aB, wvB, rnB);
-            }
-        }
-        const uint32_t any_row = row16_or(lane_bits);
-        if (col == 0 && any_row != 0u) {
-            const uint32_t lo = ((any_row & 15u) | (((any_row >> 4) & 15u) << 16)) << (4 * quad);
-            const uint32_t hi = (((any_row >> 8) & 15u) | (((any_row >> 12) & 15u) << 16)) << (4 * quad);
-            atomicOr(nl + (i - s_begin), ((unsigned long long)hi << 32) | lo);
-        }
-        st_cur = st_next; tm_cur = tm_next;
-    }
+    const int s_begin = (int)((long)n_cstages * blockIdx.y / gridDim.y);
+    const int s_end = (int)((long)n_cstages * (blockIdx.y + 1) / gridDim.y);
+    plan_walk_level1<KS32, EL>(Cst, s_begin, s_end, smem, nl, xf, xe, P);
     __syncthreads();
     for (int i = s_begin + tid; i < s_end; i += 64 * K16_NW) need[(long)blockIdx.x * n_cstages + i] = nl[i - s_begin];
     if (need2_clear != nullptr)
@@ -650,7 +663,7 @@
     const unsigned long long below = (1ull << lane) - 1ull;
     int base = 0, blk = 0, kept = 0;
     for (int s0 = 0; s0 < n_cstages; s0 += 64) {
-        const unsigned long long mine = s0 + lane < n_cstages ? need1[tile * n_cstages + s0 + lane] : 0ull;
+        const unsigned long long mine = s0 + lane < n_cstages ? need1[s0 + lane] : 0ull;
         const uint32_t lo = (uint32_t)mine, hi = (uint32_t)(mine >> 32);
         unsigned long long todo = __ballot(mine != 0ull);
         for (; todo != 0ull; todo &= todo - 1ull) {
@@ -658,7 +671,7 @@
             const unsigned long long w = ((unsigned long long)(uint32_t)__builtin_amdgcn_readlane((int)hi, sl) << 32) |
                                          (uint32_t)__builtin_amdgcn_readlane((int)lo, sl);
             uint32_t nib = 15u;
-            if (need2 != nullptr) nib = (uint32_t)(need2[tile * 4 * n_cstages + 4 * s + (lane >> 4)] >> (4 * (lane & 15))) & 15u;
+            if (need2 != nullptr) nib = (uint32_t)(need2[4 * s + (lane >> 4)] >> (4 * (lane & 15))) & 15u;
             const int g = s * 64 + lane;
             const bool l1 = ((w >> lane) & 1ull) && g < n_groups;
             const bool on = l1 && nib != 0u;
@@ -696,23 +709,25 @@
                                                          int* __restrict__ glist, int* __restrict__ gcnt,
                                                          int2* __restrict__ tile_counts, int* __restrict__ tlist,
                                                          int* __restrict__ tcnt, int* __restrict__ tile_ticket) {
-    exact_lists_tile<false>(blockIdx.x, threadIdx.x, need1, n_cstages, need2, n_groups, glist, gcnt, tile_counts, tlist, tcnt, tile_ticket);
-}
-
+    exact_lists_tile<false>(blockIdx.x, threadIdx.x, need1 + (long)blockIdx.x * n_cstages, n_cstages,
+                            need2 != nullptr ? need2 + (long)blockIdx.x * 4 * n_cstages : nullptr, n_groups, glist, gcnt, tile_counts, tlist, tcnt, tile_ticket);
+}
+
+template <int NT>
 __device__ __forceinline__ void exact_list_totals_body(const int2* tile_counts, long tiles, int* __restrict__ blocks_run,
                                                        int* __restrict__ groups_run, int slots, int2* __restrict__ items,
                                                        int* __restrict__ n_items, int* __restrict__ item_ctr, int len_pct,
                                                        int* sb, int* sk, int& tot_b) {
     const int tid = threadIdx.x, lane = tid & 63, wave = tid >> 6;
     int b = 0, k = 0;
-    for (long t = tid; t < tiles; t += 1024) { const int2 c = tile_counts[t]; b += c.x; k += c.y; }
+    for (long t = tid; t < tiles; t += NT) { const int2 c = tile_counts[t]; b += c.x; k += c.y; }
 #pragma unroll
     for (int o = 32; o > 0; o >>= 1) { b += __shfl_xor(b, o, 64); k += __shfl_xor(k, o, 64); }
     if (lane == 0) { sb[wave] = b; sk[wave] = k; }
     __syncthreads();
     if (tid == 0) {
         b = 0; k = 0;
-        for (int w = 0; w < 16; ++w) { b += sb[w]; k += sk[w]; }
+        for (int w = 0; w < NT / 64; ++w) { b += sb[w]; k += sk[w]; }
         *blocks_run = b; *groups_run = k;
         tot_b = b;
     }
@@ -722,7 +737,7 @@
     const long by_mean = (len_pct * total) / (100 * (tiles > 0 ? tiles : 1)) + 1, by_slots = total / (2 * (long)(slots > 0 ? slots : 1));
     const int L = (int)max(32L, min(by_mean, by_slots));
     auto parts_of = [&](int cnt) -> int { return cnt <= L ? 1 : (cnt + L - 1) / L; };
-    const long per = (tiles + 1023) / 1024, t_b = min((long)tid * per, tiles), t_e = min(t_b + per, tiles);
+    const long per = (tiles + NT - 1) / NT, t_b = min((long)tid * per, tiles), t_e = min(t_b + per, tiles);
     int mine = 0;
     for (long t = t_b; t < t_e; ++t) mine += parts_of(tile_counts[t].x);
     int incl = mine;
@@ -733,7 +748,7 @@
     __syncthreads();
     int before = 0, all = 0;
 #pragma unroll
-    for (int w = 0; w < 16; ++w) { if (w < wave) before += sb[w]; all += sb[w]; }
+    for (int w = 0; w < NT / 64; ++w) { if (w < wave) before += sb[w]; all += sb[w]; }
     int o = before + incl - mine;
     for (long t = t_b; t < t_e; ++t) {
         const int np = parts_of(tile_counts[t].x);
@@ -747,10 +762,31 @@
                                                                  int len_pct = 125) {
     __shared__ int sb[16], sk[16];
     __shared__ int tot_b;
-    exact_list_totals_body(tile_counts, tiles, blocks_run, groups_run, slots, items, n_items, item_ctr, len_pct, sb, sk, tot_b);
+    exact_list_totals_body<1024>(tile_counts, tiles, blocks_run, groups_run, slots, items, n_items, item_ctr, len_pct, sb, sk, tot_b);
 }
 
 constexpr int LISTS_WG_TILES = 16;
+__device__ __forceinline__ bool exact_lists_last(int* __restrict__ done, int* last_s) {
+    asm volatile("s_waitcnt vmcnt(0)" ::: "memory");
+    __syncthreads();
+    if (threadIdx.x == 0) {
+        const int ticket = __hip_atomic_fetch_add(done, 1, __ATOMIC_RELAXED, __HIP_MEMORY_SCOPE_AGENT);
+        *last_s = ticket == (int)gridDim.x - 1 ? 1 : 0;
+        if (*last_s) {
+            __builtin_amdgcn_fence(__ATOMIC_ACQUIRE, "agent");
+            asm volatile("s_waitcnt vmcnt(0)" ::: "memory");
+            __hip_atomic_store(done, 0, __ATOMIC_RELAXED, __HIP_MEMORY_SCOPE_AGENT);
+        }
+    }
+    __syncthreads();
+    return *last_s != 0;
+}
+struct PlanListsOut {
+    int n_groups;
+    int* glist; int* gcnt; int2* tile_counts; int* tlist; int* tcnt; int* tile_ticket;
+    int* done; int* blocks_run; int* groups_run;
+    int slots; int2* items; int* n_items; int* item_ctr; int len_pct;
+};
 __global__ __launch_bounds__(64 * LISTS_WG_TILES) void exact_lists_totals_kernel(const unsigned long long* __restrict__ need1, int n_cstages,
                                                                                 const unsigned long long* __restrict__ need2, int n_groups,
                                                                                 int* __restrict__ glist, int* __restrict__ gcnt,
@@ -766,21 +802,81 @@
     __shared__ int last;
     const int tid = threadIdx.x;
     const long tile = (long)blockIdx.x * LISTS_WG_TILES + (tid >> 6);
-    if (tile < tiles) exact_lists_tile<true>(tile, tid & 63, need1, n_cstages, need2, n_groups, glist, gcnt, tile_counts, tlist, tcnt, tile_ticket);
-    asm volatile("s_waitcnt vmcnt(0)" ::: "memory");
-    __syncthreads();
-    if (tid == 0) {
-        const int ticket = __hip_atomic_fetch_add(done, 1, __ATOMIC_RELAXED, __HIP_MEMORY_SCOPE_AGENT);
-        last = ticket == (int)gridDim.x - 1 ? 1 : 0;
-        if (last) {
-            __builtin_amdgcn_fence(__ATOMIC_ACQUIRE, "agent");
-            asm volatile("s_waitcnt vmcnt(0)" ::: "memory");
-            __hip_atomic_store(done, 0, __ATOMIC_RELAXED, __HIP_MEMORY_SCOPE_AGENT);
-        }
-    }
-    __syncthreads();
-    if (!last) return;
-    exact_list_totals_body(tile_counts, tiles, blocks_run, groups_run, slots, items, n_items, item_ctr, len_pct, sb, sk, tot_b);
+    if (tile < tiles)
+        exact_lists_tile<true>(tile, tid & 63, need1 + tile * n_cstages, n_cstages, need2 != nullptr ? need2 + tile * 4 * n_cstages : nullptr, n_groups,
+                               glist, gcnt, tile_counts, tlist, tcnt, tile_ticket);
+    if (!exact_lists_last(done, &last)) return;
+    exact_list_totals_body<64 * LISTS_WG_TILES>(tile_counts, tiles, blocks_run, groups_run, slots, items, n_items, item_ctr, len_pct, sb, sk, tot_b);
+}
+
+template <int KS32, class EL>
+__global__ __launch_bounds__(64 * K16_NW, 3) void exact_plan_fused_kernel(const __bf16* __restrict__ Xb, long N,
+                                                                    const char* __restrict__ Cst1, int n_cstages1, const float* __restrict__ cmax2_1,
+                                                                    const char* __restrict__ Cst2, int n_slots2, const float* __restrict__ cmax2_2,
+                                                                    const float* __restrict__ xsq, const float* __restrict__ xerr,
+                                                                    const float* __restrict__ xmax2,
+                                                                    const float* __restrict__ wmax2, const float* __restrict__ werr2,
+                                                                    ExactBound eb, const int* __restrict__ lastpos, const char* __restrict__ Wst,
+                                                                    float* __restrict__ seed_s, int force_all, PlanListsOut lo) {
+    using bf16x8 = typename V8<typename EL::T>::t;
+    constexpr int DP = 32 * KS32;
+    constexpr int STAGE = k16_stage_bytes(KS32);
+    constexpr int NT = 64 * K16_NW;
+    extern __shared__ __attribute__((aligned(16))) char smem[];
+    __shared__ int act_n;
+    __shared__ int sb_s[NT / 64], sk_s[NT / 64];
+    __shared__ int tot_b;
+    __shared__ int last;
+
+    const int tid = threadIdx.x, lane = tid & 63;
+    const int wave = __builtin_amdgcn_readfirstlane(tid >> 6);
+    const int quad = lane >> 4, col = lane & 15;
+    const long wave_s0 = (long)blockIdx.x * K16_WG_SAMPLES + wave * (16 * K16_SB);
+    const int n_cstages2 = 4 * n_cstages1;
+    int* act = (int*)(smem + 2 * STAGE);
+    unsigned long long* nl2 = (unsigned long long*)(smem + 2 * STAGE + (size_t)n_cstages1 * 64 * sizeof(int));
+    unsigned long long* nl1 = nl2 + n_cstages2;
+    float* p2s = (float*)(nl1 + n_cstages1);
+
+    bf16x8 xf[K16_SB][KS32];
+    bf16x8 xe[K16_SB];
+    float P[K16_SB];
+    {
+        const ExactScales sc1 = ex_scales(xmax2, cmax2_1, cmax2_1 + 1);
+        const ExactScales sc2 = ex_scales(xmax2, cmax2_2, cmax2_2 + 1);
+        const ExactScales sw = ex_scales(xmax2, wmax2, werr2);
+#pragma unroll
+        for (int sb = 0; sb < K16_SB; ++sb) {
+            const long row = wave_s0 + sb * 16 + col;
+#pragma unroll
+            for (int ks = 0; ks < KS32; ++ks) xf[sb][ks] = *(const bf16x8*)(Xb + row * DP + ks * 32 + quad * 8);
+            float q = 0.0f, xer = 0.0f, su = 0.0f;
+            if (row < N) {
+                q = xsq[row]; xer = xerr[row];
+                su = plan_row_seed<KS32, EL>(xf[sb], row, q, xer, eb, sw, Wst, lastpos, nullptr, nullptr, seed_s, force_all);
+            }
+            float bx1, bx2, P2;
+            plan_row_threshold<KS32>(eb, sc1, row < N, q, xer, su, P[sb], bx1);
+            plan_row_threshold<KS32>(eb, sc2, row < N, q, xer, su, P2, bx2);
+            xe[sb] = plan_extra_step<EL>(P[sb] == __builtin_inff() ? bx2 : bx1);
+            if (quad == 0) p2s[wave * (16 * K16_SB) + sb * 16 + col] = P2;
+        }
+    }
+    for (int i = tid; i < n_cstages1 + n_cstages2; i += NT) nl2[i] = 0ull;
+
+    plan_walk_level1<KS32, EL>(Cst1, 0, n_cstages1, smem, nl1, xf, xe, P);
+    __syncthreads();
+    if (wave == 0) plan_level2_list(nl1, n_cstages1, n_slots2, act, &act_n);
+#pragma unroll
+    for (int sb = 0; sb < K16_SB; ++sb) P[sb] = p2s[wave * (16 * K16_SB) + sb * 16 + col];
+    __syncthreads();
+    plan_walk_level2<KS32, EL>(Cst2, act, 0, act_n, smem, nl2, xf, xe, P);
+    __syncthreads();
+    if (wave == 0)
+        exact_lists_tile<true>(blockIdx.x, lane, nl1, n_cstages1, nl2, lo.n_groups, lo.glist, lo.gcnt, lo.tile_counts, lo.tlist, lo.tcnt, lo.tile_ticket);
+    if (!exact_lists_last(lo.done, &last)) return;
+    exact_list_totals_body<NT>(lo.tile_counts, gridDim.x, lo.blocks_run, lo.groups_run, lo.slots, lo.items, lo.n_items, lo.item_ctr, lo.len_pct,
+                               sb_s, sk_s, tot_b);
 }
 
 __global__ __launch_bounds__(256) void exact_groupkey_kernel(const int* __restrict__ g, long n, int n_groups, int* __restrict__ keys,
diff --git a/xpysom_dask_amd/csrc/somhip.hip b/xpysom_dask_amd/csrc/somhip.hip
--- a/xpysom_dask_amd/csrc/somhip.hip
+++ b/xpysom_dask_amd/csrc/somhip.hip
@@ -165,6 +165,9 @@
         DevBuf<int> tile_ticket;
         bool fuse_select = true;
         int64_t sel_fused_passes = 0, sel_launched_passes = 0, sel_ticket_tiles = 0;
+        bool fuse_plan = true;
+        int hook_plan_parts = 0;
+        int64_t plan_fused_launches = 0, plan_split_launches = 0;
         DevBuf<int2> items;
         int item_slots = 0;
         int screen_slots = 0;
@@ -1345,6 +1348,8 @@
         if (const char* e = dev_env("SOM_FUSE_MERGE")) h->fuse_merge_prep = std::atoi(e) != 0;
         if (const char* e = dev_env("SOM_EXACT_CHAIN")) h->ex.chain = std::atoi(e) != 0;
         if (const char* e = dev_env("SOM_EXACT_FUSE_SELECT")) h->ex.fuse_select = std::atoi(e) != 0;
+        if (const char* e = dev_env("SOM_EXACT_FUSE_PLAN")) h->ex.fuse_plan = std::atoi(e) != 0;
+        if (const char* e = dev_env("SOM_EXACT_PLAN_PARTS")) h->ex.hook_plan_parts = std::max(0, std::atoi(e));
         if (const char* e = dev_env("SOM_COUNTING_SORT")) h->counting_sort = std::atoi(e) != 0;
         h->use_bands = h->X > 256 || h->Y > 256;
         if (const char* e = dev_env("SOM_NO_BANDS")) h->use_bands = std::atoi(e) == 0;
@@ -2286,6 +2291,21 @@
     return 0;
 }
 
+int som_debug_exact_plan_stats(som_handle* h, int64_t* fused_launches, int64_t* split_launches) {
+    if (!h || !fused_launches || !split_launches) return fail(h, "som_debug_exact_plan_stats: NULL argument");
+    *fused_launches = h->ex.plan_fused_launches;
+    *split_launches = h->ex.plan_split_launches;
+    return 0;
+}
+
+int som_debug_exact_last_plan(som_handle* h, int32_t* out8) {
+    if (!h || !out8) return fail(h, "som_debug_exact_last_plan: NULL argument");
+    const policy::LaunchPlan& p = h->ex.lp;
+    out8[0] = p.skip; out8[1] = p.resort; out8[2] = p.scout; out8[3] = p.level2; out8[4] = p.estimate; out8[5] = p.sample_tiles;
+    out8[6] = p.refine; out8[7] = p.time_phases;
+    return 0;
+}
+
 int som_debug_qe_stats(som_handle* h, int64_t* rows, int64_t* rows_sqrt) {
     if (!h || !rows || !rows_sqrt) return fail(h, "som_debug_qe_stats: NULL argument");
     *rows = h->qe_rows;
diff --git a/xpysom_dask_amd/engine.py b/xpysom_dask_amd/engine.py
--- a/xpysom_dask_amd/engine.py
+++ b/xpysom_dask_amd/engine.py
@@ -309,6 +309,16 @@
         self._check(self._lib.som_debug_exact_select_stats(self._h, C.byref(a), C.byref(b), C.byref(c)))
         return a.value, b.value, c.value
 
+    def exact_plan_stats(self):
+        a, b = C.c_int64(), C.c_int64()
+        self._check(self._lib.som_debug_exact_plan_stats(self._h, C.byref(a), C.byref(b)))
+        return a.value, b.value
+
+    def exact_last_plan(self):
+        out = (C.c_int32 * 8)()
+        self._check(self._lib.som_debug_exact_last_plan(self._h, out))
+        return dict(zip(("skip", "resort", "scout", "level2", "estimate", "sample_tiles", "refine", "time_phases"), (bool(v) for v in out)))
+
     def exact_skip_stats(self):
         a, b = C.c_int64(), C.c_int64()
         self._check(self._lib.som_exact_skip_stats(self._h, C.byref(a), C.byref(b)))
```

Result: faster. 544.7 million (median of 6 runs) (+1.7%).
